# erincatto/solver2d

Hardware: AMD Instinct MI355X
Metric: contact-constraints x iters/sec, LargePyramid base-200 TGS_Soft (higher is better)
Workload: dtype f32

## Files before the change

include/solver2d_amd.h:

```cpp
#ifndef SOLVER2D_AMD_H
#define SOLVER2D_AMD_H

#include <stdint.h>

#ifdef __cplusplus
extern "C" {
#endif

#define S2AMD_API_VERSION 5

#define S2AMD_OK 0
#define S2AMD_E_INVALID (-1)
#define S2AMD_E_DEVICE (-2)
#define S2AMD_E_NODEVICE (-3)
#define S2AMD_E_STATE (-4)
#define S2AMD_E_CAPACITY (-5)

typedef enum s2amdSolverType
{
	s2amd_solverJacobi = 0,
	s2amd_solverPGS = 1,
	s2amd_solverPGS_NGS = 2,
	s2amd_solverPGS_NGS_Block = 3,
	s2amd_solverPGS_Soft = 4,
// ... 178 lines not shown
	uint16_t id[2];
	uint8_t cacheIndexA[3];
	uint8_t cacheIndexB[3];
	uint8_t persisted[2];
	uint8_t pad[2];
} s2amdPairState;

#define S2AMD_PAIR_UPDATED 0
#define S2AMD_PAIR_SEPARATED 1
#define S2AMD_PAIR_FREE (-1)

int s2amd_update_contacts(s2amdSolver* solver, const s2amdBody* bodies, int32_t bodyCapacity, const float* origins, const s2amdShape* shapes,
						  int32_t shapeCapacity, s2amdPairState* pairs, s2amdContact* contacts, int32_t contactCapacity, int32_t* status);

typedef struct s2amdWorldStepInfo
{
	int32_t separatedCount;
	int32_t activeContacts;
	int32_t graphChanged;
	int32_t movedCount;
	float contactsMs;
	float solveMs;
	float stepMs;
} s2amdWorldStepInfo;

int s2amd_world_upload(s2amdSolver* solver, const s2amdBody* bodies, int32_t bodyCapacity, const s2amdContact* contacts, int32_t contactCapacity,
					   const s2amdJoint* joints, int32_t jointCapacity, const s2amdShape* shapes, int32_t shapeCapacity, const s2amdPairState* pairs,
					   const float* origins);
int s2amd_world_step(s2amdSolver* solver, const s2amdStepParams* params, s2amdWorldStepInfo* info);
int s2amd_world_find_pairs(s2amdSolver* solver, int32_t* outPairs, int32_t pairCapacity, int32_t* pairCount);
int s2amd_world_separated(s2amdSolver* solver, int32_t* slots, int32_t capacity, int32_t* count);
typedef struct s2amdShapeBox
{
	float aabb[4];
	float fatAABB[4];
	int32_t enlarged;
} s2amdShapeBox;
int s2amd_world_download_boxes(s2amdSolver* solver, s2amdShapeBox* boxes, int32_t shapeCapacity);
typedef struct s2amdMovedBox
{
	int32_t shape;
	float fatAABB[4];
} s2amdMovedBox;
int s2amd_world_set_refit_order(s2amdSolver* solver, const int32_t* shapeOrder, int32_t count);
int s2amd_world_download_step(s2amdSolver* solver, float* poses, int32_t bodyCapacity, s2amdMovedBox* moved, int32_t movedCapacity, int32_t* movedCount);
typedef struct s2amdTreeNode
{
	float aabb[4];
	uint32_t categoryBits;
	int32_t parent;
	int32_t child1, child2;
	int32_t userData;
	int16_t height;
	uint8_t enlarged;
	uint8_t pad[9];
} s2amdTreeNode;
int s2amd_world_set_tree(s2amdSolver* solver, int32_t bodyType, const s2amdTreeNode* nodes, int32_t nodeCapacity, int32_t root);
int s2amd_world_get_tree(s2amdSolver* solver, int32_t bodyType, s2amdTreeNode* nodes, int32_t nodeCapacity, int32_t* root);
int s2amd_world_set_contacts(s2amdSolver* solver, const int32_t* slots, int32_t count, const s2amdContact* contacts, const s2amdPairState* pairs);
int s2amd_world_download(s2amdSolver* solver, s2amdBody* bodies, int32_t bodyCapacity, s2amdContact* contacts, int32_t contactCapacity,
						 s2amdJoint* joints, int32_t jointCapacity, s2amdShape* shapes, int32_t shapeCapacity, s2amdPairState* pairs, float* origins,
						 int32_t* status);

int s2amd_find_islands(s2amdSolver* solver, const s2amdBody* bodies, int32_t bodyCapacity, const s2amdContact* contacts, int32_t contactCapacity,
					   const s2amdJoint* joints, int32_t jointCapacity, int32_t* islandOfBody, int32_t* islandCount);
int s2amd_color_constraints(s2amdSolver* solver, const s2amdBody* bodies, int32_t bodyCapacity, const s2amdContact* contacts, int32_t contactCapacity,
							int32_t* colorOfContact, int32_t* colorCount, int32_t* rounds);

int s2amd_export_poses(s2amdSolver* solver, void* devicePoses, int32_t capacity);
int s2amd_export_poses_async(s2amdSolver* solver, void* devicePoses, int32_t capacity, int32_t slot);
int s2amd_export_bodies_async(s2amdSolver* solver, void* deviceRecords, int32_t capacity, int32_t slot);
int s2amd_export_wait(s2amdSolver* solver, int32_t slot);

int s2amd_device_alloc(s2amdSolver* solver, uint64_t bytes, void** devicePtr);
int s2amd_device_free(s2amdSolver* solver, void* devicePtr);
int s2amd_device_read(s2amdSolver* solver, void* hostDst, const void* deviceSrc, uint64_t bytes);

int s2amd_get_contact_order(s2amdSolver* solver, int32_t* order, int32_t orderCapacity, int32_t* colorOffsets,
							int32_t colorCapacity, int32_t* constraintCount, int32_t* colorCount);
int s2amd_get_joint_order(s2amdSolver* solver, int32_t* order, int32_t orderCapacity, int32_t* colorOffsets,
						  int32_t colorCapacity, int32_t* jointCount, int32_t* colorCount);
int s2amd_get_writable_bodies(s2amdSolver* solver, uint8_t* writable, int32_t bodyCapacity, int32_t* solverClass);
int s2amd_get_stats(s2amdSolver* solver, s2amdStepStats* stats);
int s2amd_get_strip_owners(s2amdSolver* solver, int32_t* ownerStrip, int32_t* onSeam, int32_t capacity, int32_t* stripCount);
int s2amd_measure_dominant(s2amdSolver* solver, const s2amdStepParams* params, int32_t repeats, float* usPerLaunch,
						   int32_t* launchesPerSweep, int32_t* constraintsPerLaunch);
int s2amd_set_option(s2amdSolver* solver, const char* key, int32_t value);

typedef struct s2amdShardedSolver s2amdShardedSolver;
int s2amd_sharded_create(const int32_t* devices, int32_t deviceCount, s2amdShardedSolver** out);
void s2amd_sharded_destroy(s2amdShardedSolver* sharded);
int s2amd_sharded_shard_count(const s2amdShardedSolver* sharded);
s2amdSolver* s2amd_sharded_solver(s2amdShardedSolver* sharded, int32_t shard);
int s2amd_sharded_upload(s2amdShardedSolver* sharded, const s2amdBody* bodies, int32_t bodyCapacity, const s2amdContact* contacts, int32_t contactCapacity,
						 const s2amdJoint* joints, int32_t jointCapacity);
int s2amd_sharded_step(s2amdShardedSolver* sharded, const s2amdStepParams* params);
int s2amd_sharded_step_async(s2amdShardedSolver* sharded, const s2amdStepParams* params);
int s2amd_sharded_wait(s2amdShardedSolver* sharded);
int s2amd_sharded_get_step_ops(s2amdShardedSolver* sharded, int32_t* streamOps, int32_t* hostWaits, int32_t* exchange);
int s2amd_sharded_count_ops(int32_t shards, int32_t exchange, int32_t* streamOps);
int s2amd_sharded_download(s2amdShardedSolver* sharded, s2amdBody* bodies, int32_t bodyCapacity, s2amdContact* contacts, int32_t contactCapacity,
						   s2amdJoint* joints, int32_t jointCapacity);
int s2amd_sharded_read_bodies(s2amdShardedSolver* sharded, int32_t shard, float* records, int32_t bodyCapacity);
int s2amd_sharded_reshard(s2amdShardedSolver* sharded, const s2amdContact* contacts, int32_t contactCapacity, const s2amdJoint* joints, int32_t jointCapacity);
int s2amd_sharded_get_partition(s2amdShardedSolver* sharded, int32_t* shardOfBody, int32_t capacity, int32_t* islandCount, int32_t* reshards);

#ifdef __cplusplus
}
#endif

#endif
```

solver2d_amd/csrc/launch.h:

```cpp
#pragma once

#include <hip/hip_runtime.h>

#include "solver2d_amd.h"

struct BodyView;
struct ContactView;
struct JointView;
struct JointPrepArgs;
struct Stage4Args;
struct StepConsts;
struct GroupTable;
struct Op;
struct MsgView;
struct StripTableView;
struct StripOps;
struct PersistView;
struct JacobiView;
struct s2amdBody;
struct s2amdContact;
struct s2amdJoint;
struct s2amdShape;
struct s2amdPairState;

// ... 56 lines not shown
						   int contactCapacity, const int* gatherIndex, const JointPrepArgs* joints = nullptr);
void launchWarmStartContacts(hipStream_t s, int kind, const ContactView& c, const BodyView& b, int begin, int end);
void launchSolveContactsSoft(hipStream_t s, int kind, const ContactView& c, const BodyView& b, int begin, int end, float inv_h, int useBias);
void launchSolveContactsRigid(hipStream_t s, int kind, const ContactView& c, const BodyView& b, int begin, int end, float inv_h);
void launchSolveContactsSticky(hipStream_t s, const ContactView& c, const BodyView& b, s2amdContact* wire, int begin, int end, float inv_h,
							   int useBias);
void launchSolveContactsNGS(hipStream_t s, const ContactView& c, const BodyView& b, int begin, int end);
void launchXpbdContactPositions(hipStream_t s, const ContactView& c, const BodyView& b, int begin, int end, float h);
void launchXpbdContactVelocities(hipStream_t s, const ContactView& c, const BodyView& b, int begin, int end, float h);
void launchBlockSolveVelocity(hipStream_t s, const ContactView& c, const BodyView& b, int begin, int end);
void launchBlockSolvePosition(hipStream_t s, const ContactView& c, const BodyView& b, int begin, int end);
bool launchStoreImpulses(hipStream_t s, int kind, const ContactView& c, s2amdContact* wire, float scale, const BodyView& bodies, s2amdBody* wireBodies,
						 void* clear, size_t clearBytes, const unsigned int* stepFailed, int finalizeMode = -1, const JointView* joints = nullptr,
						 s2amdJoint* wireJoints = nullptr,
						 const Stage4Args* stage4 = nullptr);

bool launchUnpackBodies(hipStream_t s, const BodyView& b, const s2amdBody* wire, const uint32_t* hostFlags, const StepConsts& sc, float h,
						s2amdContact* wireContacts, int contactCapacity, const int* gatherIndex, const JointPrepArgs* joints = nullptr, int posSolver = 0);
void launchPackBodies(hipStream_t s, const BodyView& b, s2amdBody* wire);
void launchIntegrateVelocities(hipStream_t s, const BodyView& b);
void launchIntegratePositions(hipStream_t s, const BodyView& b, float h);
void launchFinalizePositions(hipStream_t s, const BodyView& b, int dynamicOnly);
void launchJacobiApply(hipStream_t s, const BodyView& b, const ContactView& c, const int2* adjRange, const int* adjList, const int* heavy, int heavyCapacity);
void launchPatchWords(hipStream_t s, const void* devicePatches, int n);
void launchOverflowSweep(hipStream_t s, const Op& o, const ContactView& c, const BodyView& b, int begin, int end);
void launchXpbdIntegrate(hipStream_t s, const BodyView& b, float h);
void launchXpbdProject(hipStream_t s, const BodyView& b, float inv_h);
void launchExportPoses(hipStream_t s, const s2amdBody* wire, int n, void* out, int withVelocities = 0);

void launchPrepareJoints(hipStream_t s, int kind, const JointView& j, const uint32_t* hostFlags, const s2amdJoint* wire, const s2amdBody* wireBodies,
						 const StepConsts& sc, float h, float hertz, int warmStart, int posSolver);
void launchSolveJoints(hipStream_t s, int kind, const JointView& j, const BodyView& b, int begin, int end, const StepConsts& sc, float h,
					   float inv_h, int useBias);
void launchStoreJoints(hipStream_t s, const JointView& j, s2amdJoint* wire, const unsigned int* stepFailed);

int groupKernelSetup();
void launchGroupKernel(hipStream_t s, const ContactView& c, const JointView& j, const BodyView& g, const GroupTable& gt, const Op* ops, int opCount,
					   const StepConsts& sc, s2amdContact* wire, int maxBodies, int useDq0);
void launchStripKernel(hipStream_t s, const ContactView& c, const JointView& j, const BodyView& g, const GroupTable& gt, const Op* ops, int opCount,
					   const StepConsts& sc, s2amdContact* wire, int maxBodies, int useDq0);

void launchFillMessageSlots(hipStream_t s, const ContactView& c, const BodyView& b, const MsgView& m, int count);
void launchWarmStartContactsMsg(hipStream_t s, int kind, const ContactView& c, const MsgView& m, int begin, int end);
void launchSolveContactsSoftMsg(hipStream_t s, int kind, const ContactView& c, const MsgView& m, int begin, int end, float inv_h, int useBias);
void launchSolveContactsRigidMsg(hipStream_t s, int kind, const ContactView& c, const MsgView& m, int begin, int end, float inv_h);
void launchSolveContactsStickyMsg(hipStream_t s, const ContactView& c, const MsgView& m, s2amdContact* wire, int begin, int end, float inv_h,
								  int useBias);
void launchIntegrateVelocitiesMsg(hipStream_t s, const BodyView& b, const MsgView& m);
void launchIntegratePositionsMsg(hipStream_t s, const BodyView& b, const MsgView& m, float h);
void launchFinalizePositionsMsg(hipStream_t s, const BodyView& b, const MsgView& m, int dynamicOnly);
void launchGatherMessageSlots(hipStream_t s, const BodyView& b, const MsgView& m);

void launchWarmStartJointsBodies(hipStream_t s, const JointView& j, const BodyView& b, const int2* adjRange, const int* adjList);
void launchWarmStartBodies(hipStream_t s, int kind, const ContactView& c, const BodyView& b, const int2* adjRange, const int* adjList,
						   int integrateFirst, const int* heavy, int heavyCount);

int stripKernelSetup();
void launchIslandStep(hipStream_t s, int kind, int warm, const ContactView& c, const BodyView& g, const StripTableView& t, const float4* softCoef, const Op* ops,
					  int opCount, int maxRounds, s2amdContact* wire, const s2amdBody* wireBodies, const uint32_t* hostFlags, int warmStart,
					  const unsigned int* stepFailed);
void launchStripSoft(hipStream_t s, int kind, int warm, const ContactView& c, const BodyView& g, const StripTableView& t, const StripOps& ops);
void launchStripStep(hipStream_t s, int kind, int warm, const ContactView& c, const BodyView& g, const StripTableView& a, const PersistView& pv,
					 const Op* ops, int opCount);

int pairKernelSetup();
void launchPairStep(hipStream_t s, int kind, int warm, const ContactView& c, const BodyView& g, const StripTableView& a, const PersistView& pv, const Op* ops,
					int opCount);

int wideKernelSetup();
struct WideSelf
{
	s2amdContact* wire;
	s2amdBody* wireBodies;
	const uint32_t* hostFlags;
	int warmStart;
	float gravityX, gravityY, unpackH;
};
int wideExtraRecords(const PersistView& pv, int selfContained, int bodyWarm, int kind = SOFT_TGS);
int wideBodyWarmVariant(const PersistView& pv);
int wideIslandLocalRecords(int maxRounds);
void launchWideIsland(hipStream_t s, const ContactView& c, const BodyView& g, const StripTableView& t, const float4* softCoef, const Op* ops, int opCount,
					  int maxRounds, s2amdContact* wire, s2amdBody* wireBodies, const uint32_t* hostFlags, int warmStart, const StepConsts& sc, float unpackH,
					  int selfContained, const unsigned int* stepFailed, int allTwoPoints);
void launchWideStep(hipStream_t s, int kind, const ContactView& c, const BodyView& g, const StripTableView& a, const PersistView& pv, const Op* ops, int opCount,
					const WideSelf* self);

int jacobiKernelSetup();
size_t jacobiStepLds(int owned, int imports, int constraints, int opCount);
void launchJacobiStep(hipStream_t s, const ContactView& c, const JointView& jv, const BodyView& g, const JacobiView& t, const Op* ops, int opCount, const StepConsts& sc,
					  size_t ldsBytes, int maxConstraints);

int genericKernelSetup();
size_t genericStepLds(int bodies, int seamBodies, int exports, int opCount, int useDq0, int stagedJoints = 0);
void launchGenericStep(hipStream_t s, const ContactView& c, const JointView& j, const BodyView& g, const GroupTable& a, const GroupTable& b, const PersistView& pv,
					   const Op* ops, int opCount, const StepConsts& sc, s2amdContact* wire, int useDq0, int seamContacts, int seamJoints, size_t ldsBytes,
					   int stageJoints);

void launchUpdateContacts(hipStream_t st, const s2amdBody* bodies, const float* origins, const s2amdShape* shapes, s2amdPairState* pairs,
						  s2amdContact* contacts, int contactCapacity, int32_t* status, uint8_t* pointBytes, int* summary, int* separatedSlots, const uint8_t* watched);
void launchStage4(hipStream_t st, s2amdBody* bodies, int bodyCapacity, s2amdShape* shapes, int shapeCapacity, float* origins, int* summary,
				  const unsigned int* stepFailed = nullptr);
struct TreeView
{
	s2amdTreeNode* nodes;
	int* flag;
	int* leaves;
	int* state;
	int capacity;
	int *acc, *pending, *oldPre, *leafIdx, *partner, *arrive;
	float *cx, *cy;
	int *tasks, *ready, *qstate;
};
struct TreeViews
{
	TreeView t[3];
	const int* refitPos;
};
struct DeviceTrees;
void treesFree(s2amdSolver* s);
void treesForget(s2amdSolver* s);
bool treesActive(const s2amdSolver* s);
const TreeViews* treesViews(const s2amdSolver* s);
int treesSyncRefitOrder(s2amdSolver* s);
int worldWarmPairQuery(s2amdSolver* s);
void launchTreeEnlarge(s2amdSolver* s, hipStream_t st, const unsigned int* stepFailed);
void launchTreeRebuild(s2amdSolver* s, hipStream_t st);
void treesJoin(s2amdSolver* s, hipStream_t st);
void launchOrderPairs(hipStream_t st, const TreeViews* views, const s2amdShape* shapes, const unsigned char* moved, const unsigned long long* keys,
					  const unsigned int* count, unsigned int cap, unsigned long long* ckeys, unsigned long long* out);
struct PairQueryGraph
{
	hipGraphExec_t exec = nullptr;
	unsigned long long key = 0, keySeen = 0;
	bool disabled = false;
	char* host = nullptr;
	void* countAt = nullptr;
	size_t outCapWanted = 0;
};
struct PairQueryHook
{
	void (*fn)(void* arg, hipStream_t st);
	void* arg;
};
int findPairsResident(hipStream_t st, const s2amdShape* shapes, int shapeCapacity, int liveShapes, const s2amdPairState* pairs, int contactCapacity,
					  const unsigned long long* jointed, int jointedCount, int32_t* outPairs, int32_t pairCapacity, int32_t* pairCount, void** scratch,
					  size_t* scratchBytes, unsigned long long* sortedPairKeys, bool* sortedPairKeysValid, PairQueryGraph* cache, int mode = 0,
					  const unsigned long long* pairLog = nullptr, const int* pairLogSlots = nullptr, const TreeViews* trees = nullptr,
					  const PairQueryHook* hook = nullptr);
#define S2_PAIR_LOG_ENTRIES 255
#define S2_PAIRS_FULL 0
#define S2_PAIRS_WARM 1
#define S2_PAIRS_ENQUEUE 2
#define S2_PAIRS_COLLECT 3

#define S2_DEFINE_WARM(name)                                                                                                     \
	__global__ void s2WarmKernel_##name() {}                                                                                    \
	void s2Warm_##name(hipStream_t st) { s2WarmKernel_##name<<<dim3(1), dim3(64), 0, st>>>(); }
void s2Warm_contact_kernels(hipStream_t st);
void s2Warm_body_kernels(hipStream_t st);
void s2Warm_joint_kernels(hipStream_t st);
void s2Warm_group_kernel(hipStream_t st);
void s2Warm_strip_kernel(hipStream_t st);
void s2Warm_pair_kernel(hipStream_t st);
void s2Warm_wide_kernel(hipStream_t st);
void s2Warm_generic_kernel(hipStream_t st);
void s2Warm_broadphase(hipStream_t st);
void s2Warm_narrowphase(hipStream_t st);
// ... 7 lines not shown
```

solver2d_amd/csrc/s2_device.h:

```cpp
#pragma once

#include <hip/hip_runtime.h>
#include <stdint.h>

#define S2_DEV __device__ __forceinline__

#define S2_PI 3.14159265359f
#define S2_LINEAR_SLOP 0.005f
#define S2_ANGULAR_SLOP (2.0f / 180.0f * S2_PI)
#define S2_MAX_LINEAR_CORRECTION 0.2f
#define S2_MAX_ANGULAR_CORRECTION (8.0f / 180.0f * S2_PI)
#define S2_BAUMGARTE 0.2f
#define S2_MAX_BAUMGARTE_VELOCITY 4.0f
#define S2_CONTACT_HERTZ 30.0f
#define S2_JOINT_HERTZ 60.0f

#define S2_MINF(A, B) ((A) < (B) ? (A) : (B))
#define S2_MAXF(A, B) ((A) > (B) ? (A) : (B))
#define S2_ABSF(A) ((A) > 0.0f ? (A) : -(A))
#define S2_CLAMPF(A, B, C) S2_MINF(S2_MAXF(A, B), C)

struct V2
{
	float x, y;
// ... 391 lines not shown
struct GroupTable
{
	const int* bodyOffsets;
	const int* bodyIds;
	const int* cBatchOffsets;
	const int4* cBatches;
	const int* jBatchOffsets;
	const int4* jBatches;
	int groupCount;
};
#define S2G_OWNED 0x80000000u

#define S2_STRIP_ROUNDS 6
#define S2_STRIP_ROUNDS_MAX 8
#define S2_STRIP_BODY_CHUNKS 4
struct StripDesc
{
	int bodyBase, bodyCount, ownedCount;
	int batchCount;
	int slotBase, slotCount, slotOffBase;
	int pad;
	int4 batch[S2_STRIP_ROUNDS_MAX];
};
struct StripOps
{
	int integratePos, integrateVel, sweep, useBias;
	float posH, inv_h;
};
struct StripTableView
{
	const StripDesc* descs;
	const int* bodyIds;
	const int2* slots;
	const int* slotOffsets;
	int groupCount;
	int ldsRecords;
};

#define S2_PERSIST_B_ROUNDS 4
#define S2_PERSIST_Q_NARROW 6
#define S2_PERSIST_Q_WIDE 8
struct PersistDesc
{
	int importCount[2];
	int importIdBase[2];
	int exportCount[2];
	int exportSrcBase[2];
	int inBase[2];
	int outBase[2];
	int remapBase[2];
	int seamBatchCount[2];
	int2 seamBatch[2][S2_PERSIST_B_ROUNDS];
	int seamGroup[2];
	int pad[6];
};
struct PersistView
{
	const PersistDesc* descs;
	const int* remap;
	const int* exportSrc;
	const int* importIds;
	unsigned long long* granules;
	unsigned int* error;
	unsigned int* deviceError;
	int parityStride;
	int censusBase;
	int allTwoPoints;
	float4 softCoef[2];
	int wideRounds;
	int seamRegs;
	int maxRoundsA, maxSeamRounds;
	int pairLanes;
	int nearHandoff;
	int wideOnly;
	int ldsRecords;
	int parkSeamWidth, parkInteriorWidth;
	int bodyRecords;
	int debugSkip;
	unsigned int spinLimit;
	unsigned int* state;
	int maxStaged;
	int maxStripBodies;
	int bodyWarm;
	int clearOwn;
	const int* overflowBodies;
	int overflowBodyCount;
	int overflowBegin, overflowEnd;
	int overflowGranBase;
	int overflowKernel;
	unsigned long long* debugTimes;
};
#define S2_OVERFLOW_BODIES 64
#define S2_OVERFLOW_RING 4
#define S2_OVERFLOW_GRANULES (2 * S2_OVERFLOW_RING * S2_OVERFLOW_BODIES * 4)

#define S2_JACOBI_HEAVY 32
struct JacobiBlockDesc
{
	int ownedBase, ownedCount;
	int importBase, importCount;
	int constraintBase, constraintCount;
	int listBase, rangeBase;
	int exportBase, exportCount;
	int heavyBase, heavyCount;
	int jointBase, jointCount;
};
struct JacobiView
{
	const JacobiBlockDesc* descs;
	const int* ints;
	unsigned long long* granules;
	int parityStride;
	unsigned int* error;
	unsigned int* deviceError;
	unsigned int spinLimit;
	int blockCount;
	int debugSkip;
};

struct MsgView
{
	float4* vel;
	float4* dq;
	const int* next;
	const int* firstSlot;
	const int* slotOffsets;
	const int* slotList;
};
```

solver2d_amd/csrc/solver.cpp:

```cpp

#include <atomic>
#include "solver_executor.h"

namespace
{

thread_local std::string g_lastError;

}

int s2amdFail(int code, const std::string& msg)
{
	g_lastError = msg;
	return code;
}

hipStream_t s2amdStream(s2amdSolver* s)
{
	return s->stream;
}
void s2amdRecordDeviceMs(s2amdSolver* s, float ms)
{
	s->stats.deviceMs = ms;
}
// ... 553 lines not shown
		return fail(S2AMD_E_CAPACITY, "the solver holds " + std::to_string(s->hBodyFlags.size()) + " bodies");
	}
	const int cls = s->orderSolverClass == 1 ? 1 : 0;
	const uint32_t bit = cls == 1 ? S2F_WRITE_POS : S2F_WRITE_VEL;
	for (size_t i = 0; i < s->hBodyFlags.size(); ++i)
	{
		writable[i] = (s->hBodyFlags[i] & bit) != 0 ? 1 : 0;
	}
	if (solverClass)
	{
		*solverClass = cls;
	}
	return S2AMD_OK;
}

int s2amd_get_joint_order(s2amdSolver* s, int32_t* order, int32_t orderCapacity, int32_t* colorOffsets, int32_t colorCapacity, int32_t* jointCount,
						  int32_t* colorCount)
{
	if (!s)
	{
		return fail(S2AMD_E_INVALID, "null solver");
	}
	return copyOrder(s->joints.order, s->joints.colorOffsets, order, orderCapacity, colorOffsets, colorCapacity, jointCount, colorCount);
}

int s2amd_get_strip_owners(s2amdSolver* s, int32_t* ownerStrip, int32_t* onSeam, int32_t capacity, int32_t* stripCount)
{
	if (!s)
	{
		return fail(S2AMD_E_INVALID, "null solver");
	}
	const IncrementalStrips& m = s->stripInc;
	const int nb = s->bodyCapacity;
	if ((ownerStrip || onSeam) && capacity < nb)
	{
		return fail(S2AMD_E_CAPACITY, "strip owner buffer too small");
	}
	if (stripCount)
	{
		*stripCount = m.valid ? (int)m.stripBodyCount.size() : 0;
	}
	for (int i = 0; i < nb; ++i)
	{
		if (ownerStrip)
		{
			ownerStrip[i] = (m.valid && i < (int)m.ownerStrip.size()) ? m.ownerStrip[(size_t)i] : -1;
		}
		if (onSeam)
		{
			onSeam[i] = -1;
		}
	}
	if (onSeam && m.valid)
	{
		for (size_t sm = 0; sm < m.seamGroupOf.size(); ++sm)
		{
			const int g = m.seamGroupOf[sm];
			if (g < 0)
			{
				continue;
			}
			for (const auto& kv : m.seamSlot[(size_t)g])
			{
				if (kv.first >= 0 && kv.first < nb && m.ownerStrip[(size_t)kv.first] >= 0)
				{
					onSeam[kv.first] = (int)sm;
				}
			}
		}
	}
	return S2AMD_OK;
}

int s2amd_get_stats(s2amdSolver* s, s2amdStepStats* stats)
{
	if (!s || !stats)
	{
		return fail(S2AMD_E_INVALID, "null argument");
	}
	*stats = s->stats;
	return S2AMD_OK;
}

int s2amd_export_poses(s2amdSolver* s, void* devicePoses, int32_t capacity)
{
	if (!s || !s->resident)
	{
		return fail(S2AMD_E_STATE, "nothing resident");
	}
	if (!devicePoses || capacity < s->bodyCapacity)
	{
		return fail(S2AMD_E_CAPACITY, "pose buffer missing or too small");
	}
	HIP_TRY(hipSetDevice(s->device));
	launchExportPoses(s->stream, (const s2amdBody*)s->dBodies.p, s->bodyCapacity, devicePoses);
	HIP_TRY(hipGetLastError());
	HIP_TRY(hipStreamSynchronize(s->stream));
	return S2AMD_OK;
}

int s2amd_export_poses_async(s2amdSolver* s, void* devicePoses, int32_t capacity, int32_t slot)
{
	if (!s || !s->resident)
	{
		return fail(S2AMD_E_STATE, "nothing resident");
	}
	if (!devicePoses || capacity < s->bodyCapacity || slot < 0 || slot >= 4)
	{
		return fail(S2AMD_E_CAPACITY, "pose buffer missing or too small, or slot outside 0..3");
	}
	HIP_TRY(hipSetDevice(s->device));
	if (!s->evExport[slot])
	{
		HIP_TRY(hipEventCreateWithFlags(&s->evExport[slot], hipEventDisableTiming));
	}
	launchExportPoses(s->stream, (const s2amdBody*)s->dBodies.p, s->bodyCapacity, devicePoses);
	HIP_TRY(hipGetLastError());
	HIP_TRY(hipEventRecord(s->evExport[slot], s->stream));
	return S2AMD_OK;
}

int s2amd_export_bodies_async(s2amdSolver* s, void* deviceRecords, int32_t capacity, int32_t slot)
{
	if (!s || !s->resident)
	{
		return fail(S2AMD_E_STATE, "nothing resident");
	}
	if (!deviceRecords || capacity < s->bodyCapacity || slot < 0 || slot >= 4)
	{
		return fail(S2AMD_E_CAPACITY, "record buffer missing or too small, or slot outside 0..3");
	}
	HIP_TRY(hipSetDevice(s->device));
	if (!s->evExport[slot])
	{
		HIP_TRY(hipEventCreateWithFlags(&s->evExport[slot], hipEventDisableTiming));
	}
	launchExportPoses(s->stream, (const s2amdBody*)s->dBodies.p, s->bodyCapacity, deviceRecords, 1);
	HIP_TRY(hipGetLastError());
	HIP_TRY(hipEventRecord(s->evExport[slot], s->stream));
	return S2AMD_OK;
}

int s2amd_export_wait(s2amdSolver* s, int32_t slot)
{
	if (!s || slot < 0 || slot >= 4 || !s->evExport[slot])
	{
		return fail(S2AMD_E_STATE, "no export recorded in this slot");
	}
	HIP_TRY(hipSetDevice(s->device));
	HIP_TRY(hipEventSynchronize(s->evExport[slot]));
	return S2AMD_OK;
}

int s2amd_device_alloc(s2amdSolver* s, uint64_t bytes, void** devicePtr)
{
	if (!s || !devicePtr)
	{
		return fail(S2AMD_E_INVALID, "null argument");
	}
	*devicePtr = nullptr;
	HIP_TRY(hipSetDevice(s->device));
	HIP_TRY(hipMalloc(devicePtr, bytes > 0 ? (size_t)bytes : 16));
	HIP_TRY(hipMemsetAsync(*devicePtr, 0, bytes > 0 ? (size_t)bytes : 16, s->stream));
	HIP_TRY(hipStreamSynchronize(s->stream));
	return S2AMD_OK;
}
// ... 266 lines not shown
	}
	else if (strcmp(key, "strip_retry") == 0)
	{
		s->optStripRetry = value != 0;
		s->structureDirty = true;
	}
	else if (strcmp(key, "persist") == 0)
	{
		s->stripsRejected = false;
		s->optPersist = value != 0;
		s->structureDirty = true;
	}
	else if (strcmp(key, "strip_patience") == 0)
	{
		s->optStripPatience = std::max(0, value);
		s->stripPatienceNow = s->optStripPatience;
		s->stripPatienceSet = true;
	}
	else if (strcmp(key, "near_handoff") == 0)
	{
		s->optNearHandoff = value != 0;
		s->nearHandoffNow = s->optNearHandoff;
	}
	else if (strcmp(key, "strip_adopt") == 0)
	{
		s->optStripAdopt = value != 0;
	}
	else if (strcmp(key, "prebuild_solver") == 0)
	{
		s->optPrebuildSolver = value;
	}
	else if (strcmp(key, "jacobi_persist") == 0)
	{
		s->optJacobiPersist = value != 0;
		s->structureDirty = true;
	}
	else if (strcmp(key, "jacobi_min_constraints") == 0)
	{
		s->optJacobiMinConstraints = std::max(0, value);
		s->structureDirty = true;
	}
	else if (strcmp(key, "strip_overflow") == 0)
	{
		s->optOverflow = value != 0;
		s->structureDirty = true;
	}
	else if (strcmp(key, "cost_strip_round_ns") == 0 || strcmp(key, "cost_launch_ns") == 0 || strcmp(key, "cost_tail_visit_ns") == 0)
	{
		float& f = key[5] == 's' ? s->hubCosts.stripRoundUs : (key[5] == 'l' ? s->hubCosts.launchUs : s->hubCosts.tailVisitUs);
		f = 1e-3f * (float)std::max(value, 1);
		s->structureDirty = true;
	}
	else if (strcmp(key, "tree_stream") == 0)
	{
		s->optTreeStream = value != 0 ? 1 : 0;
	}
	else if (strcmp(key, "pairs_in_step") == 0)
	{
		s->optPairsInStep = value != 0;
		s->pairCacheValid = false;
	}
	else if (strcmp(key, "overflow_kernel") == 0)
	{
		s->optOverflowKernel = value != 0;
		s->overflowKernelFailed = false;
		s->layoutGeneration += 1;
	}
	else if (strcmp(key, "stage_joints") == 0)
	{
		s->optStageJoints = value != 0;
	}
	else if (strcmp(key, "step_readback") == 0)
	{
		s->optStepReadback = value != 0;
	}
	else if (strcmp(key, "self_contained") == 0)
	{
		s->optSelfContained = value != 0;
	}
	else if (strcmp(key, "strip_body_warm") == 0)
	{
		s->optWideBodyWarm = value != 0;
	}
	else if (strcmp(key, "self_contained_strips") == 0)
	{
		if (s->optSelfContainedStrips != (value != 0 ? 1 : 0))
		{
			s->structureDirty = true;
		}
		s->optSelfContainedStrips = value != 0;
	}
	else if (strcmp(key, "free_body_groups") == 0)
	{
		s->optFreeBodyGroups = value != 0;
		s->structureDirty = true;
	}
	else if (strcmp(key, "persist_retry") == 0)
	{
		s->optPersistRetry = std::max(0, value);
		s->persistRetryAfter = std::max(1, value);
	}
	else if (strcmp(key, "generic") == 0)
	{
		s->stripsRejected = false;
		s->optGeneric = value != 0;
		s->structureDirty = true;
	}
	else if (strcmp(key, "strips_any_solver") == 0)
	{
		s->stripsRejected = false;
		s->optStripsAnySolver = value != 0;
		s->structureDirty = true;
	}
	else if (strcmp(key, "island_resident") == 0)
	{
		s->optIslandResident = value != 0;
		s->residentRejected = false;
		s->structureDirty = true;
	}
	else if (strcmp(key, "incremental") == 0)
	{
		s->optIncremental = value != 0;
		s->structureDirty = true;
	}
	else if (strcmp(key, "defer") == 0)
	{
		s->optDefer = value != 0;
		s->structureDirty = true;
	}
	else if (strcmp(key, "strip_lean") == 0)
	{
		s->stripsRejected = false;
		s->optStripLean = value != 0;
		s->structureDirty = true;
	}
	else if (strcmp(key, "strip_bodies") == 0)
	{
		s->stripsRejected = false;
		s->optStripBodies = std::max(1, value);
		s->stripBodiesSet = true;
		s->structureDirty = true;
	}
	else if (strcmp(key, "strip_min_bodies") == 0)
	{
		s->stripsRejected = false;
		s->optStripMinBodies = std::max(0, value);
		s->stripMinBodiesSet = true;
		s->structureDirty = true;
	}
	else if (strcmp(key, "pack_group_bodies") == 0)
	{
		s->optPackGroupBodies = std::max(1, value);
		s->packGroupBodiesSet = true;
		s->structureDirty = true;
	}
	else
	{
		return fail(S2AMD_E_INVALID, std::string("unknown option ") + key);
	}
	return S2AMD_OK;
}

}
#pragma GCC visibility pop
```

solver2d_amd/csrc/solver_executor.h:

```cpp
#pragma once

#include "solver_internal.h"


struct Executor
{
	s2amdSolver* s;
	hipStream_t st;
	const StepPlan& p;
	int posSolver;
	bool profile;
	bool msg = false;
	bool fork = false;
	const int* gatherIndex = nullptr;

	hipStream_t branch(int i, int forkEvent)
	{
		if (!fork)
		{
			return st;
		}
		(void)hipEventRecord(s->evFork[forkEvent], st);
		(void)hipStreamWaitEvent(s->side[i], s->evFork[forkEvent], 0);
		return s->side[i];
// ... 336 lines not shown
				continue;
			}
			if (o.code == OP_WARM && (o.kind == WARM_CURRENT || o.kind == WARM_FIXED) && (warm < 0 || warm == o.kind))
			{
				warm = o.kind;
				continue;
			}
			if (leanSoftKind(o) && (kind < 0 || kind == o.kind))
			{
				kind = o.kind;
				continue;
			}
			return false;
		}
		if (kind < 0)
		{
			return false;
		}
		if (warm < 0)
		{
			warm = kind == SOFT_FIXED ? WARM_FIXED : WARM_CURRENT;
		}
		if (widePlan(kind, warm))
		{
			return true;
		}
		if (s->persist.wideOnly)
		{
			return false;
		}
		const bool narrow = kind == SOFT_TGS && warm == WARM_CURRENT;
		const int records = (narrow ? s->persist.ldsRecords : s->persistRecordsWide) + 2 * (int)p.ops.size();
		return records <= (160 * 1024) / 16;
	}

	bool genericPlan() const
	{
		if (!s->genericValid || s->persistFailed || p.ops.size() > 128)
		{
			return false;
		}
		for (const Op& o : p.ops)
		{
			if (o.code == OP_JACOBI_APPLY || (o.code == OP_SOLVE_SOFT && o.kind == SOFT_JACOBI))
			{
				return false;
			}
		}
		return genericStepLds(s->genericBodies, s->genericSeamBodies, s->genericExports, (int)p.ops.size(), p.usesDq0 ? 1 : 0) <= 160 * 1024;
	}

	bool oneLaunchPlan() const
	{
		int kind, warm;
		return persistPlan(kind, warm) || genericPlan();
	}

	bool widePlan(int kind, int warm) const
	{
		const bool current = (kind == SOFT_TGS || kind == SOFT_PGS) && warm == WARM_CURRENT;
		const bool fixed = kind == SOFT_FIXED && warm == WARM_FIXED;
		return s->optWide && (current || fixed) && wideFits(false, false, kind);
	}

	bool wideFits(bool selfContained, bool bodyWarm, int kind = SOFT_TGS) const
	{
		const int extra = wideExtraRecords(s->persist, selfContained ? 1 : 0, bodyWarm ? 1 : 0, kind);
		return extra >= 0 && s->persist.bodyRecords + 3 + extra + 2 * s->persistOpCount <= (160 * 1024) / 16;
	}

	bool selfContainedStrips() const
	{
		int kind, warm;
		return s->optSelfContainedStrips && !slicedPlan() && s->dStripA.view.groupCount > 0 && persistPlan(kind, warm) && kind == SOFT_TGS && widePlan(kind, warm) && wideFits(true, false) && gatherIndex == nullptr && !msg &&
			   wireBodies() != nullptr && s->dGroups.view.groupCount == 0 && s->dResident.view.groupCount == 0 && s->looseBodies == 0 && !anyGlobalContacts() &&
			   s->joints.globalCount == 0 && s->jv.count == 0 && s->cv.count == s->persistK1 - s->persistK0 && p.prepContacts == PREP_SOFT && p.storeKind == STORE_PLAIN;
	}

	bool wideBodyWarm(bool selfContained) const
	{
		return s->optWideBodyWarm != 0 && wideBodyWarmVariant(s->persist) != 0 && wideFits(selfContained, true);
	}

	bool residentPlan(int& kind, int& warm) const
	{
		kind = -1, warm = -1;
		if (s->residentView.groupCount <= 0 || p.ops.size() > 128 || p.prepContacts != PREP_SOFT || p.storeKind != STORE_PLAIN)
		{
			return false;
		}
		if (s->dStripA.view.groupCount > 0 && oneLaunchPlan())
		{
			return false;
		}
		for (const Op& o : p.ops)
		{
			if (o.code == OP_INTEGRATE_VEL || o.code == OP_INTEGRATE_POS || o.code == OP_FINALIZE || o.code == OP_JOINT_SWEEP)
			{
				continue;
			}
			if (o.code == OP_WARM && (o.kind == WARM_CURRENT || o.kind == WARM_FIXED) && (warm < 0 || warm == o.kind))
			{
				warm = o.kind;
				continue;
			}
			if (leanSoftKind(o) && (kind < 0 || kind == o.kind))
			{
				kind = o.kind;
				continue;
			}
			return false;
		}
		if (kind < 0)
		{
			return false;
		}
		if (warm < 0)
		{
			warm = kind == SOFT_FIXED ? WARM_FIXED : WARM_CURRENT;
		}
		return true;
	}

	int uploadResidentOps()
	{
		if (s->residentOpsGeneration == s->planGeneration)
		{
			return 0;
		}
		std::vector<Op> kept;
		for (const Op& o : p.ops)
		{
			if (o.code != OP_JOINT_SWEEP)
			{
				kept.push_back(o);
			}
		}
		bool grew = false;
		int rc = s->dResidentOps.ensure(std::max<size_t>(kept.size(), 1) * sizeof(Op), &grew);
		if (rc)
		{
			return rc;
		}
		if (grew)
		{
			s->layoutGeneration += 1;
		}
		if (hipMemcpyAsync(s->dResidentOps.p, kept.data(), kept.size() * sizeof(Op), hipMemcpyHostToDevice, st) != hipSuccess ||
			hipStreamSynchronize(st) != hipSuccess)
		{
			return S2AMD_E_DEVICE;
		}
		s->residentOpCount = (int)kept.size();
		s->residentOpsGeneration = s->planGeneration;
		return 0;
	}

	bool wideIslandPlan() const
	{
		int kind, warm;
		return residentPlan(kind, warm) && s->optWide && kind == SOFT_TGS && warm == WARM_CURRENT &&
			   s->residentView.ldsRecords + 2 + wideIslandLocalRecords(s->residentRounds) + 2 * s->residentOpCount <= (160 * 1024) / 16;
	}

	bool selfContainedIslands() const
	{
// ... 21 lines not shown
			{
				launchWideIsland(st, s->cv, s->bv, s->residentView, coef, (const Op*)s->dResidentOps.p, s->residentOpCount, s->residentRounds, wireContacts(),
								 wireBodies(), (const uint32_t*)s->dBodyFlags.p, p.sc.warmStart, p.sc, p.unpackH, selfContained ? 1 : 0, stepFailed,
								 (s->residentAllTwoPoints && s->pointsKnown) ? 1 : 0);
			}
			else
			{
				launchIslandStep(st, kind, warm, s->cv, s->bv, s->residentView, coef, (const Op*)s->dResidentOps.p, s->residentOpCount, s->residentRounds,
								 wireContacts(), wireBodies(), (const uint32_t*)s->dBodyFlags.p, p.sc.warmStart, stepFailed);
			}
		}
		else
		{
			launchGroupKernel(st, s->cv, s->jv, s->bv, s->dResident.view, deviceOps(), (int)p.ops.size(), p.sc, wireContacts(), s->dResident.maxBodies,
							  p.usesDq0 ? 1 : 0);
		}
		count();
	}

	int uploadPersistOps()
	{
		if (s->persistOpsGeneration == s->planGeneration && s->persistOpsStructure == s->structureGeneration)
		{
			return 0;
		}
		std::vector<Op> kept;
		for (const Op& o : p.ops)
		{
			if (!sweepsNothing(o))
			{
				kept.push_back(o);
			}
		}
		bool grew = false;
		int rc = s->dPersistOps.ensure(std::max<size_t>(kept.size(), 1) * sizeof(Op), &grew);
		if (rc)
		{
			return rc;
		}
		if (grew)
		{
			s->layoutGeneration += 1;
		}
		if (hipMemcpyAsync(s->dPersistOps.p, kept.data(), kept.size() * sizeof(Op), hipMemcpyHostToDevice, st) != hipSuccess ||
			hipStreamSynchronize(st) != hipSuccess)
		{
			return S2AMD_E_DEVICE;
		}
		s->persistOpCount = (int)kept.size();
		s->persistOpsGeneration = s->planGeneration;
		s->persistOpsStructure = s->structureGeneration;
		return 0;
	}

	std::vector<Op> keptOps() const
	{
		std::vector<Op> kept;
		for (const Op& o : p.ops)
		{
			if (!sweepsNothing(o))
			{
				kept.push_back(o);
			}
		}
		return kept;
	}

	bool slicedPlan() const { return s->stripInc.valid && s->stripInc.overflowUsed > 0; }

	void runPersistentSliced(int kind, int warm)
	{
		const std::vector<Op> kept = keptOps();
		const int n = (int)kept.size();
		PersistView pv = s->persist;
		pv.nearHandoff = s->nearHandoffNow;
		for (int i = 0; i < 2; ++i)
		{
			pv.softCoef[i] = make_float4(p.sc.softCoef[i][0], p.sc.softCoef[i][1], p.sc.softCoef[i][2], 0.0f);
		}
		if (!(kind == SOFT_TGS && warm == WARM_CURRENT))
		{
			pv.ldsRecords = s->persistRecordsWide;
		}
		pv.bodyWarm = 0;
		pv.clearOwn = 1;
		const IncrementalStrips& m = s->stripInc;
		int first = 0;
		for (int i = 0; i < n; ++i)
		{
			const Op& o = kept[(size_t)i];
			const bool sweep = o.code == OP_WARM || leanSoftKind(o);
			if (!sweep && i + 1 < n)
			{
				continue;
			}
			launchWideStep(st, kind, s->cv, s->bv, s->leanA, pv, (const Op*)s->dPersistOps.p + first, i + 1 - first, nullptr);
			count();
			if (sweep)
			{
				launchOverflowSweep(st, o, s->cv, s->bv, m.overflowBegin, m.overflowEnd);
				count();
			}
			first = i + 1;
		}
	}

	void clearGranules(hipStream_t where)
	{
		(void)hipMemsetAsync(s->dGranules.p, 0, s->granuleBytes, where);
		count();
	}

	bool overflowKernelPlan() const
	{
		return slicedPlan() && s->optOverflowKernel != 0 && !s->overflowKernelFailed && s->persist.overflowBodies != nullptr && s->dStripA.view.groupCount + 1 <= s->cuCount;
	}

	void runPersistent(int kind, int warm, bool clearFirst = false, bool selfContained = false, bool overflowKernel = false)
	{
		if (clearFirst)
		{
			clearGranules(st);
		}
		if (profile)
		{
			recordEvent();
		}
		PersistView pv = s->persist;
		pv.nearHandoff = s->nearHandoffNow;
		for (int i = 0; i < 2; ++i)
		{
			pv.softCoef[i] = make_float4(p.sc.softCoef[i][0], p.sc.softCoef[i][1], p.sc.softCoef[i][2], 0.0f);
		}
		if (!(kind == SOFT_TGS && warm == WARM_CURRENT))
		{
			pv.ldsRecords = s->persistRecordsWide;
		}
		if (widePlan(kind, warm))
		{
			WideSelf self{};
			if (selfContained)
			{
				self.wire = wireContacts(), self.wireBodies = wireBodies(), self.hostFlags = (const uint32_t*)s->dBodyFlags.p;
				self.warmStart = p.sc.warmStart, self.gravityX = p.sc.gravityX, self.gravityY = p.sc.gravityY, self.unpackH = p.unpackH;
			}
			pv.bodyWarm = (kind == SOFT_TGS && wideBodyWarm(selfContained)) ? 1 : 0;
			if (overflowKernel)
			{
				const IncrementalStrips& m = s->stripInc;
				pv.bodyWarm = 0;
				pv.overflowKernel = 1;
				pv.overflowBodyCount = (int)m.overflowBodyIds.size();
				pv.overflowBegin = m.overflowBegin, pv.overflowEnd = m.overflowEnd;
			}
			launchWideStep(st, kind, s->cv, s->bv, s->leanA, pv, (const Op*)s->dPersistOps.p, s->persistOpCount, selfContained ? &self : nullptr);
		}
		else if (pv.pairLanes && s->optPairLanes)
		{
			launchPairStep(st, kind, warm, s->cv, s->bv, s->leanA, pv, (const Op*)s->dPersistOps.p, s->persistOpCount);
		}
		else
		{
			launchStripStep(st, kind, warm, s->cv, s->bv, s->leanA, pv, (const Op*)s->dPersistOps.p, s->persistOpCount);
		}
		if (profile)
		{
			recordEvent();
		}
		count();
	}

	void runGeneric()
	{
		if (profile)
		{
			recordEvent();
		}
		const size_t withJoints = genericStepLds(s->genericBodies, s->genericSeamBodies, s->genericExports, s->persistOpCount, p.usesDq0 ? 1 : 0, s->genericJoints);
		const bool stage = s->optStageJoints != 0 && s->genericJoints > 0 && withJoints <= 160 * 1024;
		const size_t lds = stage ? withJoints : genericStepLds(s->genericBodies, s->genericSeamBodies, s->genericExports, s->persistOpCount, p.usesDq0 ? 1 : 0);
		PersistView gpv = s->persist;
		gpv.nearHandoff = s->nearHandoffNow;
		launchGenericStep(st, s->cv, s->jv, s->bv, s->dStripA.view, s->dStripB.view, gpv, (const Op*)s->dPersistOps.p, s->persistOpCount, p.sc,
						  wireContacts(), p.usesDq0 ? 1 : 0, s->contacts.seamCount > 0 ? 1 : 0, s->joints.seamCount > 0 ? 1 : 0, lds, stage ? 1 : 0);
		if (profile)
		{
			recordEvent();
		}
		count();
	}

	void runStrips()
	{
		int kind, warm;
		if (persistPlan(kind, warm))
		{
			if (slicedPlan() && widePlan(kind, warm))
			{
				if (overflowKernelPlan())
				{
					runPersistent(kind, warm, false, false, true);
				}
				else
				{
					runPersistentSliced(kind, warm);
				}
			}
			else
			{
				runPersistent(kind, warm);
			}
			return;
		}
		if (genericPlan())
		{
			runGeneric();
			return;
		}
		const int n = (int)p.ops.size();
		int segStart = 0;
		for (int i = 0; i < n; ++i)
		{
			const Op& o = p.ops[(size_t)i];
			if (isBodyOp(o.code) || sweepsNothing(o))
			{
				continue;
			}
			StripOps lean;
			int warm = -1;
			if (o.code == OP_WARM)
			{
				int j = i + 1;
				while (j < n && (isBodyOp(p.ops[(size_t)j].code) || sweepsNothing(p.ops[(size_t)j])))
				{
					j += 1;
				}
				if (j < n && leanSegment(segStart, j, lean, warm) && warm >= 0)
				{
// ... 224 lines not shown
```

solver2d_amd/csrc/solver_internal.h:

```cpp
#pragma once

#include "launch.h"
#include "s2_device.h"

#include "solver2d_amd.h"

#include <algorithm>
#include <chrono>
#include <cmath>
#include <cstdio>
#include <cstdlib>
#include <cstring>
#include <string>
#include <unordered_map>
#include <vector>

int s2amdFail(int code, const std::string& msg);
inline int fail(int code, const std::string& msg) { return s2amdFail(code, msg); }

#define S2_HUB_DEGREE 12
#define S2_COST_STRIP_ROUND_US 1.4f
#define S2_COST_LAUNCH_US 2.0f
#define S2_COST_BATCH_COLOURS 12
#define S2_COST_TAIL_VISIT_US 0.38f
// ... 200 lines not shown
	bool takeOnly = false;
	std::vector<int> stripBodyBase, stripBodyCount;
	std::vector<int> stripListCapacity;
	std::vector<std::vector<int>> movedList;
	std::vector<int> adoptedBy;
	int spareIdsNext = 0, spareIdsEnd = 0;
	long adopted = 0;
	std::vector<int> seamBodyCount;
	std::vector<int> seamExtra[2];
	long seamBodiesAdded = 0;
	int overflowBegin = 0, overflowEnd = 0;
	std::vector<int> overflowFree;
	int overflowUsed = 0;
	long overflowPlaced = 0;
	std::vector<int> overflowBodyIds;
};
#define S2_OVERFLOW_SLACK 32
#define S2_STRIP_ADOPT_SLACK 8
#define S2_TAIL_SLACK 64
#define S2_GROUP_PATIENCE_MIN_POSITIONS 16384
#define S2_TAIL_BODY_SLACK 32

struct SolverStructure
{
	std::vector<int> hContactA, hContactB;
	std::vector<uint8_t> hContactEdge;
	std::vector<uint8_t> hContactDead;
	std::vector<uint8_t> hBodyHub, hContactWatched;
	int watchedCount = 0;
	DevBuf dWatched;
	std::vector<uint32_t> hBodyFlagsFinal;
	std::vector<uint8_t> hBodyLdsOwned;
	DevBuf dBodyFlags;

	DevBuf soaBodies, soaContacts, soaJoints, dContactIndex, dJointIndex, dContactLocal, dJointLocal, dAdjOffsets, dAdjList, dAdjHeavy;
	int adjHeavyCapacity = 0;
	IncrementalGlobal inc;
	uint4* hostPatches = nullptr;
	size_t hostPatchCapacity = 0;
	DevBuf dPatches;
	int spareColours = 0;
	DevBuf dJointAdjRange, dJointAdjList;
	bool jointAdjValid = false;
	int slackPositions = 0;
	bool slackBumped = false;
	int slackAtBuild = 0;
	int slackShift = 0;
	const char* dirtyReason = "";
	bool watchedDirty = false;
	BodyView bv{};
	ContactView cv{};
	JointView jv{};
	uint64_t layoutGeneration = 0;
	int bodySoaCap = 0, contactSoaCap = 0, jointSoaCap = 0;

	SweepSet contacts, joints;
	HostGroupTable hGroups, hContactTail, hJointTail, hStripA, hStripB;
	std::vector<int> hPersistRemap;
	std::vector<PersistDesc> hPersistDescs;
	DeviceGroupTable dGroups, dContactTail, dJointTail, dStripA, dStripB;
	HostGroupTable hResident;
	DeviceGroupTable dResident;
	DevBuf dResidentDesc, dResidentOps;
	StripTableView residentView{};
	int residentRounds = 0;
	int residentK0 = 0, residentK1 = 0;
	bool residentRejected = false;
	uint64_t residentOpsGeneration = ~0ull;
	int residentOpCount = 0;
	DevBuf dStripLean;
	StripTableView leanA{}, leanB{};
	bool leanAValid = false, leanBValid = false;
	DevBuf dPersist, dGranules, dOverflowBodies;
	PersistView persist{};
	bool persistValid = false;
	bool genericValid = false;
	int genericJoints = 0;
	int genericBodies = 0, genericSeamBodies = 0, genericExports = 0;
	int residentAllTwoPoints = 0;
	int persistK0 = 0, persistK1 = 0;
	int persistRecordsWide = 0;
	DevBuf dPersistOps;
	int persistOpCount = 0;
	DevBuf dJacobi, dJacobiGran;
	JacobiView jacobi{};
	int jacobiDeferred = 0;
	bool jacobiValid = false;
	size_t jacobiGranBytes = 0;
	int jacobiMaxOwned = 0, jacobiMaxImports = 0, jacobiMaxConstraints = 0;
	uint64_t persistOpsGeneration = ~0ull, persistOpsStructure = ~0ull;
	size_t granuleBytes = 0;
	long selfStepsSinceReset = 0;
	IncrementalStrips stripInc;
	float stripScaleFound = 0.0f;
	bool stripRetryPending = false;
	DevBuf dMsg;
	MsgView msg{};
	bool msgTablesValid = false;
	int looseBodies = 0;
	int orderSolverClass = -1;
	bool orderGrouped = false;
	bool orderLdsGroups = false;
	bool orderResident = false;
	bool orderColourless = false;
	bool orderStrips = false;
	int orderStripBodies = 0;
	bool stripsNeedOneLaunch = false;
	bool stripsRejected = false;
	int stripsJudgedForClass = -1;
	bool stripsHopeless = false;
	bool adjValid = false;
	bool structureDirty = true;
	uint64_t structureGeneration = 0;
	int stripScaleFoundFor = 0;

	hipGraph_t graph = nullptr;
	hipGraphExec_t graphExec = nullptr;
	uint64_t graphKey = 0;
	uint64_t graphKeySeen = 0;
	int graphKeySeenLaunches = 0;
	int graphLaunches = 0;
};

struct AsyncBuild;

struct SolverRest
{
	int device = 0;
	hipStream_t stream = nullptr;
	hipEvent_t evBegin = nullptr, evEnd = nullptr;
	hipEvent_t evExport[4] = {nullptr, nullptr, nullptr, nullptr};
	hipStream_t side[2] = {nullptr, nullptr};
	hipEvent_t evFork[2] = {nullptr, nullptr}, evJoin[4] = {nullptr, nullptr, nullptr, nullptr};
	int optAsync = 0;
	bool constraintIndexInPrologue = false;
	int optFork = 0;

	DevBuf dBodies, dContacts, dJoints, dBodiesSaved;
	int bodyCapacity = 0, contactCapacity = 0, jointCapacity = 0;
	bool resident = false;
	bool savedValid = false;
	int savedBodyCapacity = 0;

	DevBuf dShapes, dPairs, dOrigins, dStatus, dPointBytes, dWorldSummary, dJointedKeys, dContactStage, dPairScratch, dPairKeys;
	PairQueryGraph pairQuery;
	bool pairKeysValid = false;
	int shapeCapacity = 0, liveShapes = 0, jointedCount = 0;
	bool worldResident = false;
	int* hostWorldSummary = nullptr;
	uint8_t* hostSlotStage = nullptr;
	size_t hostSlotStageBytes = 0;
	char* hostStepBack = nullptr;
	size_t hostStepBackBytes = 0, stepBackPoseOffset = 0;
	int stepBackBoxes = 0;
	bool stepBackValid = false;
	bool stepBackListFresh = false;
	int optStepReadback = 1;
	std::vector<uint8_t> hPointBytes;
	std::vector<uint8_t> hShapeMovable;
	int movableShapes = 0;
	std::vector<int> hContactPoints;
	bool deadUnknown = false;
	bool pointsKnown = false;
	bool pointCountsFresh = false;
	int optPrebuildSolver = -1;
	int activeContacts = 0;
	bool lastStepWroteIndex = false;
	DevBuf dScanTmp;
	std::vector<int> hJointType, hJointA, hJointB;
	std::vector<uint32_t> hBodyFlags;
	std::vector<uint8_t> hBodyLive, hBodyStatic;
	DevBuf dOps;
	long placedTotal = 0;
	DevBuf dSeparated;
	DevBuf dPairLog;
	unsigned long long* hostPairLog = nullptr;
	bool pairLogDirty = false;
	DevBuf dShapeBoxes;
	DevBuf dRefitOrder, dStepBack;
	int refitOrderCount = 0;
	int optTreeStream = 1;
	DeviceTrees* trees = nullptr;
	int lastMovedCount = 0;
	DevBuf dSlotBytes;
	std::vector<uint8_t> hSlotBytes;
	bool slotBytesFresh = false;
	std::vector<int32_t> hSeparated;
	int optIncremental = 1;
	int optDefer = 1;
	int optIslandResident = 1;
	int optStripLean = 1;
	int optStageJoints = 1;
	int optSelfContained = 1;
	int optGeneric = 1;
	int optFreeBodyGroups = 1;
	int optPersist = 1;
	int optSeamRegs = 1;
	int optWide = 1;
	int optWideBodyWarm = 0;
	int optSelfContainedStrips = 0;
	int optStripSlack = 1;
	int optPairLanes = 0;
	int optStripRetry = 1;
	int optPersistDebug = 0;
	int optPersistSpinLimit = 1 << 21;
	bool persistFailed = false;
	int persistFallbacks = 0;
	int optPersistRetry = 256;
	int persistRetryAfter = 256, persistFailedAge = 0;
	int cuCount = 0;
	HubCosts hubCosts;
	unsigned int* hostError = nullptr;
	unsigned long long* hostTimes = nullptr;
	int optMessage = 0;
	int optBodyWarm = 1;
	bool indexInWire = false;
	int graphAge = 0;
	int optStripPatience = 1;
	int optNearHandoff = 1, nearHandoffNow = 1, nearHandoffTimeouts = 0;
	int optStripAdopt = 1;
	int optJacobiPersist = 1;
	int optJacobiMinConstraints = 1024;
	int optOverflow = 1;
	long slicedSteps = 0;
	bool slicedThisStep = false;
	int stripPatienceNow = 1;
	int groupPatienceNow = 0;
	bool dirtyByGroups = false;
	int tailSlackShift = 0;
	bool dirtyByWatched = false;
	int optGroupPatience = 1;
	int optTailTinyColour = 32;
	int optGroupTinyColour = 3;
	int optGenericPlace = 1;
	int optFlipColours = 1;
	bool stripPatienceSet = false;
	int optStripsAnySolver = 0;

	StepPlan plan;
	uint64_t planGeneration = 0;

	int optGraph = 1;
	int optGraphMinLaunches = 6;
	int optProfile = 0;
	int optGroups = 1;
	int optMaxGroupBodies = 1024;
	bool maxGroupBodiesSet = false;
	int optPackGroupBodies = 1024;
	bool packGroupBodiesSet = false;
	int optStrips = 1;
	int optStripBodies = 8;
	bool stripBodiesSet = false;
	int optStripBodiesLds = 320;
	bool stripMinBodiesSet = false;
	int optStripMinBodies = 768;

	std::vector<hipEvent_t> sweepEvents;
	size_t sweepEventsUsed = 0;

	s2amdStepStats stats{};
	int launchCounter = 0;
	DevBuf dGatherIndex;
	bool gatherIndexDirty = true;
	uint64_t opsGeneration = ~0ull;

	AsyncBuild* async = nullptr;
	int optAsyncBuild = 1;
	int optAsyncBuildDelay = 12;
	bool isClone = false;
	bool poolWarmed = false;
	bool forcedBuild = false;
	Stage4Args stage4{};
	bool stage4Carried = false;
	bool graphCarriesStage4 = false;
	int optPairsInStep = 1;
	bool pairQueryUsed = false;
	bool pairCacheValid = false;
	int optOverflowKernel = 1;
	bool overflowKernelFailed = false;
	bool overflowKernelThisStep = false;
	int overflowRefusals = 0;
	long stepCounter = 0;
// ... 120 lines not shown
```

solver2d_amd/csrc/solver_step.cpp:

```cpp
#include "solver_executor.h"

void destroyGraph(s2amdSolver* s)
{
	if (s->graphExec)
	{
		(void)hipGraphExecDestroy(s->graphExec);
		s->graphExec = nullptr;
	}
	if (s->graph)
	{
		(void)hipGraphDestroy(s->graph);
		s->graph = nullptr;
	}
	s->graphKey = 0;
}

int resetPersistState(s2amdSolver* s, hipStream_t st)
{
	if (s->hostError)
	{
		*s->hostError = 0u;
	}
	if (s->persist.deviceError)
	{
// ... 575 lines not shown
		}
		if ((key != s->graphKey || s->graphExec == nullptr) && (key != s->graphKeySeen || s->graphKeySeenLaunches < s->optGraphMinLaunches))
		{
			s->graphKeySeen = key;
			q.fork = false;
			enqueueAll();
			s->graphKeySeenLaunches = s->launchCounter;
		}
		else if (key != s->graphKey || s->graphExec == nullptr)
		{
			destroyGraph(s);
			HIP_TRY(hipStreamBeginCapture(s->stream, hipStreamCaptureModeThreadLocal));
			enqueueAll();
			hipError_t ce = hipStreamEndCapture(s->stream, &s->graph);
			if (ce != hipSuccess)
			{
				s->graph = nullptr;
				return fail(S2AMD_E_DEVICE, std::string("hipStreamEndCapture: ") + hipGetErrorString(ce));
			}
			HIP_TRY(hipGraphInstantiate(&s->graphExec, s->graph, nullptr, nullptr, 0));
			s->graphKey = key;
			s->graphLaunches = s->launchCounter;
			s->graphCarriesStage4 = s->stage4Carried;
		}
		else
		{
			s->launchCounter = s->graphLaunches;
			s->stats.graphReplayed = 1;
			s->stage4Carried = s->graphCarriesStage4;
		}
		if (key == s->graphKey && s->graphExec != nullptr)
		{
			HIP_TRY(hipGraphLaunch(s->graphExec, s->stream));
		}
	}
	else
	{
		enqueueAll();
	}
	HIP_TRY(hipEventRecord(s->evEnd, s->stream));
	HIP_TRY(hipGetLastError());
	s->indexInWire = s->indexInWire || indexNow;
	const bool async = s->optAsync != 0 && !q.profile;
	if (!async)
	{
		HIP_TRY(hipStreamSynchronize(s->stream));
		float ms = 0.0f;
		HIP_TRY(hipEventElapsedTime(&ms, s->evBegin, s->evEnd));
		s->stats.deviceMs = ms;
	}
	s->stats.constraintCount = s->activeContacts;
	s->stats.jointCount = s->jv.count;
	s->stats.contactColors = (int)s->contacts.colorOffsets.size() - 1;
	s->stats.jointColors = (int)s->joints.colorOffsets.size() - 1;
	s->stats.solveSweeps = plan.solveSweeps;
	s->stats.kernelLaunches = s->launchCounter;
	s->stats.groupCount = s->dGroups.view.groupCount + s->dResident.view.groupCount;
	s->stats.stripCount = s->dStripA.view.groupCount;
	s->stats.seamCount = s->dStripB.view.groupCount;
	{
		int kind, warm;
		s->stats.persistent = ((s->dStripA.view.groupCount > 0 && (q.persistPlan(kind, warm) || q.genericPlan())) || q.jacobiPlan()) ? 1 : 0;
	}
	s->stats.persistFallbacks = s->persistFallbacks;
	s->stats.asyncBuildsRequested = s->asyncRequested, s->stats.asyncBuildsAdopted = s->asyncAdopted, s->stats.asyncWaitMs = s->asyncWaitMs;
	s->stats.nearHandoffTimeouts = s->nearHandoffTimeouts;
	{
		int kind, warm;
		s->slicedThisStep = s->dStripA.view.groupCount > 0 && q.slicedPlan() && q.persistPlan(kind, warm) && q.widePlan(kind, warm) && !q.selfContainedStrips();
		s->overflowKernelThisStep = s->slicedThisStep && q.overflowKernelPlan();
		s->slicedSteps += s->slicedThisStep ? 1 : 0;
		s->stats.overflowContacts = s->stripInc.valid ? s->stripInc.overflowUsed : 0;
		s->stats.slicedStep = s->slicedThisStep ? (s->overflowKernelThisStep ? 2 : 1) : 0;
		s->stats.slicedSteps = (int32_t)s->slicedSteps;
	}
	s->stats.bodiesAdopted = (int32_t)s->stripInc.adopted, s->stats.seamBodiesAdded = (int32_t)s->stripInc.seamBodiesAdded, s->stats.roundsOpened = (int32_t)s->stripInc.roundsOpened;
	s->stats.structureBuilds = (int32_t)s->structureGeneration;
	s->stats.placedContacts = (int32_t)s->placedTotal;
	{
		int kind = -1, warm = -1;
		const bool persistent = s->stats.persistent && q.persistPlan(kind, warm);
		const bool wide = persistent && q.widePlan(kind, warm);
		s->stats.pairLanes = wide ? 2 : (persistent && s->persist.pairLanes && s->optPairLanes) ? 1 : (s->stats.persistent && !persistent) ? 3 : 0;
	}
	s->stats.potentialConstraints = (int32_t)(s->contacts.order.size() - (size_t)s->slackPositions);
	if (!async && s->hostError && *s->hostError != 0u)
	{
		int rcReset = resetPersistState(s, s->stream);
		if (rcReset)
		{
			return rcReset;
		}
		if (s->nearHandoffNow != 0 && s->stats.persistent)
		{
			s->nearHandoffNow = 0;
			s->nearHandoffTimeouts += 1;
			s->layoutGeneration += 1;
			s->stepCounter -= 1;
			return doStep(s, params);
		}
		if (s->overflowKernelThisStep && !s->overflowKernelFailed)
		{
			s->overflowKernelFailed = true;
			s->layoutGeneration += 1;
			s->persistFallbacks += 1;
			s->stepCounter -= 1;
			return doStep(s, params);
		}
		s->persistFailed = true;
		s->persistFailedAge = 0;
		s->persistFallbacks += 1;
		s->stepCounter -= 1;
		return doStep(s, params);
	}
	s->graphAge += 1;
	if (q.profile)
	{
		float total = 0.0f;
		for (size_t i = 0; i + 1 < s->sweepEventsUsed; i += 2)
		{
			float t = 0.0f;
			if (hipEventElapsedTime(&t, s->sweepEvents[i], s->sweepEvents[i + 1]) == hipSuccess)
			{
				total += t;
			}
		}
		float empty = 0.0f;
		int pairs = 0;
		if (s->sweepEvents.size() >= 2)
		{
			for (int r = 0; r < 32; ++r)
			{
				(void)hipEventRecord(s->sweepEvents[0], s->stream);
				(void)hipEventRecord(s->sweepEvents[1], s->stream);
				(void)hipStreamSynchronize(s->stream);
				float t = 0.0f;
				if (hipEventElapsedTime(&t, s->sweepEvents[0], s->sweepEvents[1]) == hipSuccess)
				{
					empty += t;
					pairs += 1;
				}
			}
		}
		s->stats.solveKernelMs = total;
		s->stats.solveLaunches = (int)(s->sweepEventsUsed / 2);
		s->stats.eventPairOverheadMs = pairs > 0 ? empty / pairs : 0.0f;
	}
	return S2AMD_OK;
}

int doDownload(s2amdSolver* s, s2amdBody* bodies, int nb, s2amdContact* contacts, int nc, s2amdJoint* joints, int nj)
{
	if (!s->resident)
	{
		return fail(S2AMD_E_STATE, "nothing resident to download");
	}
	if (nb < s->bodyCapacity || nc < s->contactCapacity || nj < s->jointCapacity)
	{
		return fail(S2AMD_E_CAPACITY, "output arrays smaller than the resident world");
	}
	HIP_TRY(hipSetDevice(s->device));
	if (contacts && !s->pointsKnown && s->lastStepWroteIndex)
	{
		int rc = refreshConstraintIndexOnDevice(s);
		if (rc)
		{
// ... 20 lines not shown
```

solver2d_amd/csrc/wide_kernel.hip:

```cpp

#include "body_ops.h"
#include "persist_handoff.h"
#include "soft_from_wire.h"

#ifndef S2_PERSIST_INSTRUMENTED
#define S2_PERSIST_INSTRUMENTED 0
#endif
#ifndef S2_WIDE_XCD_AFFINE
#define S2_WIDE_XCD_AFFINE 1
#endif
#define S2_WIDE_THREADS 512
#define S2_WIDE_INTERIOR 256
#define S2_WIDE_ROUNDS_PER_HALF (S2_STRIP_ROUNDS / 2)
#define S2_WIDE_BODY_CHUNKS 2
#define S2_WIDE_SEAM_ROUNDS 2

typedef float f2 __attribute__((ext_vector_type(2)));

S2_DEV f2 lo2(float4 v) { return f2{v.x, v.y}; }
S2_DEV f2 hi2(float4 v) { return f2{v.z, v.w}; }
struct WideRegs
{
	uint32_t idx;
	f2 n;
// ... 375 lines not shown
			const float tangentMass = fromBits(asBits(p.p2[j]) ^ salt);
			const V2 rA = pre.rA[j], rB = pre.rB[j];
			const V2 vrB = add(vB, crossSV(wB, rB));
			const V2 vrA = add(vA, crossSV(wA, rA));
			const float vt = dot(sub(vrB, vrA), tangent);
			float impulse = -tangentMass * vt;
			const float maxFriction = p.friction * nImp[j];
			const float newImpulse = S2_CLAMPF(tImp[j] + impulse, -maxFriction, maxFriction);
			impulse = newImpulse - tImp[j];
			const V2 P = mulSV(impulse, tangent);
			vA = mulSub(vA, mA, P);
			wA -= iA * cross(rA, P);
			vB = mulAdd(vB, mB, P);
			wB += iB * cross(rB, P);
			p.imp[j] = f2{nImp[j], newImpulse};
		}
	}

	if ((idx & (1u << 28)) != 0)
	{
		lvel[ia] = make_float4(vA.x, vA.y, wA, 0.0f);
	}
	if ((idx & (1u << 29)) != 0)
	{
		lvel[ib] = make_float4(vB.x, vB.y, wB, 0.0f);
	}
}
#endif

S2_DEV void storeWide(const ContactView& c, const WideRegs& p, int k)
{
	const int pointCount = (int)((p.idx >> 26) & 3u);
#pragma unroll
	for (int j = 0; j < 2; ++j)
	{
		if (j < pointCount)
		{
			c.impulse[j][k] = make_float2(p.imp[j].x, p.imp[j].y);
		}
	}
}

#define S2_WIDE_PARKED_RECORDS 6
#ifndef S2_WIDE_PARKED_PREP_EARLY
#define S2_WIDE_PARKED_PREP_EARLY 0
#endif
S2_DEV void parkWide(float4* slot, int stride, const WideRegs& p)
{
	slot[0 * stride] = make_float4(fromBits(p.idx), p.n.x, p.n.y, p.friction);
	slot[1 * stride] = make_float4(p.lA[0].x, p.lA[0].y, p.lA[1].x, p.lA[1].y);
	slot[2 * stride] = make_float4(p.lB[0].x, p.lB[0].y, p.lB[1].x, p.lB[1].y);
	slot[3 * stride] = make_float4(p.p0[0], p.p0[1], p.p1[0], p.p1[1]);
	slot[4 * stride] = make_float4(p.p2[0], p.p2[1], 0.0f, 0.0f);
	slot[5 * stride] = make_float4(p.imp[0].x, p.imp[0].y, p.imp[1].x, p.imp[1].y);
}
S2_DEV WideRegs unparkWide(const float4* slot, int stride)
{
	const float4 q0 = slot[0 * stride], q1 = slot[1 * stride], q2 = slot[2 * stride], q3 = slot[3 * stride], q4 = slot[4 * stride], q5 = slot[5 * stride];
	WideRegs p;
	p.idx = asBits(q0.x), p.n = f2{q0.y, q0.z}, p.friction = q0.w;
	p.lA[0] = lo2(q1), p.lA[1] = hi2(q1), p.lB[0] = lo2(q2), p.lB[1] = hi2(q2);
	p.p0[0] = q3.x, p.p0[1] = q3.y, p.p1[0] = q3.z, p.p1[1] = q3.w, p.p2[0] = q4.x, p.p2[1] = q4.y;
	p.imp[0] = lo2(q5), p.imp[1] = hi2(q5);
	return p;
}

S2_DEV WideRegs wideFromSoft(const SoftRegs<SOFT_TGS>& t)
{
	WideRegs p;
	p.idx = (uint32_t)t.h.ia | ((uint32_t)t.h.ib << 13) | (((uint32_t)t.h.pointCount & 3u) << 26) | (t.h.writeA ? 1u << 28 : 0u) | (t.h.writeB ? 1u << 29 : 0u);
	p.n = f2{t.h.normal.x, t.h.normal.y}, p.friction = t.h.friction;
#pragma unroll
	for (int j = 0; j < 2; ++j)
	{
		p.lA[j] = lo2(t.an[j]), p.lB[j] = hi2(t.an[j]);
		p.p0[j] = t.par[j].x, p.p1[j] = t.par[j].y, p.p2[j] = t.par[j].z;
		p.imp[j] = f2{t.imp[j].x, t.imp[j].y};
	}
	return p;
}

#define S2_WIDE_SELF 1
#define S2_WIDE_BODYWARM 2
#define S2_WIDE_SLICED 4

template <int POINTS, bool LL = false>
S2_DEV void warmTermsWide(const WideRegs& p, const float4* ldq, const float2* lmass, float2* lt, int tw, int R, int round, int nOwn, uint32_t salt, const float4* locals = nullptr)
{
	const uint32_t idx = p.idx ^ salt;
	const int ia = (int)(idx & 0x1fffu), ib = (int)((idx >> 13) & 0x1fffu);
	const int pointCount = (int)((idx >> 26) & 3u);
	const bool wa = (idx & (1u << 28)) != 0 && ia < nOwn, wb = (idx & (1u << 29)) != 0 && ib < nOwn;
	const float4 dqA = ldq[ia], dqB = ldq[ib];
	const float2 mA = lmass[ia], mB = lmass[ib];
	const V2 normal = v2(fromBits(asBits(p.n.x) ^ salt), p.n.y);
	const V2 tangent = rightPerp(normal);
	Rot qA, qB;
	qA.s = dqA.z, qA.c = dqA.w, qB.s = dqB.z, qB.c = dqB.w;
	float tA[6], tB[6];
#pragma unroll
	for (int j = 0; j < 2; ++j)
	{
		tA[3 * j] = tA[3 * j + 1] = tA[3 * j + 2] = 0.0f;
		tB[3 * j] = tB[3 * j + 1] = tB[3 * j + 2] = 0.0f;
		if (POINTS == 2 || j < pointCount)
		{
			V2 lAj, lBj;
			if constexpr (LL)
			{
				const float4 a = locals[j * S2_WIDE_THREADS];
				lAj = v2(a.x, a.y), lBj = v2(a.z, a.w);
			}
			else
			{
				lAj = asV2(p.lA[j]), lBj = asV2(p.lB[j]);
			}
			const V2 rA = rotate(qA, lAj), rB = rotate(qB, lBj);
			const V2 P = add(mulSV(p.imp[j].x, normal), mulSV(p.imp[j].y, tangent));
			tA[3 * j] = -mA.x * P.x, tA[3 * j + 1] = -mA.x * P.y, tA[3 * j + 2] = -(mA.y * cross(rA, P));
			tB[3 * j] = mB.x * P.x, tB[3 * j + 1] = mB.x * P.y, tB[3 * j + 2] = mB.y * cross(rB, P);
		}
	}
	float2* row = lt + (size_t)round * tw;
	const int plane = R * tw;
	if (wa)
	{
		row[ia] = make_float2(tA[0], tA[1]);
		row[plane + ia] = make_float2(tA[2], tA[3]);
		row[2 * plane + ia] = make_float2(tA[4], tA[5]);
	}
	if (wb)
	{
		row[ib] = make_float2(tB[0], tB[1]);
		row[plane + ib] = make_float2(tB[2], tB[3]);
		row[2 * plane + ib] = make_float2(tB[4], tB[5]);
	}
}

constexpr int wideLocalsInLds(int RPH, int SR, int SL, int IL, bool sliced)
{
	const int plain = (SL > 0 || IL > 0) ? (IL > 0 ? 4 : 3) : ((RPH + SR > 5) ? 3 : 0);
	return plain > 0 && sliced ? plain + 1 : plain;
}

S2_DEV int wideOverflowExchange(const PersistView& pv, const int* lovf, float4* lvel, int ovCount, unsigned sweep)
{
	const int tid = (int)threadIdx.x;
	int fail = 0;
	if (tid < ovCount)
	{
		const int e = lovf[tid];
		if (e != 0)
		{
			const int slot = e & 0xffffff;
			gu64* in = (gu64*)pv.granules + pv.overflowGranBase + (int)(sweep & (S2_OVERFLOW_RING - 1)) * S2_OVERFLOW_BODIES * 4 + 4 * tid;
			gu64* out = in + S2_OVERFLOW_GRANULES / 2;
			if ((e >> 24) == 3)
			{
				const float4 v = lvel[slot];
				putGranule(in + 0, sweep, v.x), putGranule(in + 1, sweep, v.y), putGranule(in + 2, sweep, v.z);
			}
			float v[3];
			if (getGranules<3>(out, sweep, v, pv.error, pv.deviceError, pv.spinLimit))
			{
				lvel[slot] = make_float4(v[0], v[1], v[2], 0.0f);
			}
			else
			{
				fail = 1;
			}
		}
	}
	return __syncthreads_or(fail);
}

#define S2_WIDE_OVERFLOW 8

template <int KIND> S2_DEV void wideOverflowWorker(const ContactView& c, const BodyView& g, const PersistView& pv, const Op* ops, int opCount, float4* lds)
{
	const int tid = (int)threadIdx.x;
	const int M = pv.overflowBodyCount;
	__shared__ float4 lvel[S2_OVERFLOW_BODIES], ldq[S2_OVERFLOW_BODIES];
	Op* lops = (Op*)lds;
	uint32_t flags = 0u;
	bool exchanged = false;
	float4 vel = make_float4(0.0f, 0.0f, 0.0f, 0.0f), dq = vel, integ = vel;
	float angDamp = 0.0f;
	if (tid < M)
	{
		const int e = pv.overflowBodies[tid];
		if (e >= 0)
		{
			const int gi = e & 0x3fffffff;
			exchanged = (e & 0x40000000) == 0;
			vel = g.vel[gi], dq = g.dq[gi], integ = g.integ[gi], angDamp = g.angDamp[gi];
			flags = g.flags[gi];
		}
	}
	for (int i = tid; i < opCount * 8; i += S2_WIDE_THREADS)
	{
		((int*)lops)[i] = ((const int*)ops)[i];
	}
	const int myK = pv.overflowBegin + tid;
	const bool mine = tid < 64 && myK < pv.overflowEnd && c.contactIndex[myK] >= 0;
	__syncthreads();
	const LdsBodies lb{lvel, ldq};
	gu64* in = (gu64*)pv.granules + pv.overflowGranBase + 4 * tid;
	gu64* out = in + S2_OVERFLOW_GRANULES / 2;
	unsigned sweep = 0u;
	for (int oi = 0; oi < opCount; ++oi)
	{
		const Op op = lops[oi];
		if (op.code == OP_INTEGRATE_VEL)
		{
			if ((flags & S2F_DYNAMIC) != 0)
			{
				V2 lv = add(v2(vel.x, vel.y), v2(integ.x, integ.y));
				float w = vel.z + integ.z;
				lv = mulSV(integ.w, lv);
				w *= angDamp;
				vel = make_float4(lv.x, lv.y, w, 0.0f);
// ... 59 lines not shown
					__builtin_amdgcn_fence(__ATOMIC_RELEASE, "wavefront");
					__builtin_amdgcn_wave_barrier();
					__builtin_amdgcn_fence(__ATOMIC_ACQUIRE, "wavefront");
				}
			}
			__syncthreads();
			if (exchanged)
			{
				vel = lvel[tid];
				putGranule(out + ring + 0, sweep, vel.x), putGranule(out + ring + 1, sweep, vel.y), putGranule(out + ring + 2, sweep, vel.z);
			}
		}
		else if (op.code == OP_WARM)
		{
			WarmRegs w;
			if (mine)
			{
				w = op.kind == WARM_FIXED ? loadWarm<WARM_FIXED>(c, lb, myK) : loadWarm<WARM_CURRENT>(c, lb, myK);
			}
			sweep += 1u;
			const int ring = (int)(sweep & (S2_OVERFLOW_RING - 1)) * S2_OVERFLOW_BODIES * 4;
			int fail = 0;
			if (exchanged)
			{
				float v[3];
				if (getGranules<3>(in + ring, sweep, v, pv.error, pv.deviceError, pv.spinLimit))
				{
					vel = make_float4(v[0], v[1], v[2], 0.0f);
				}
				else
				{
					fail = 1;
				}
			}
			if (tid < M)
			{
				lvel[tid] = vel, ldq[tid] = dq;
			}
			if (__syncthreads_or(fail))
			{
				return;
			}
			if (tid < 64)
			{
				for (unsigned long long turns = __ballot(mine); turns != 0ull; turns &= turns - 1ull)
				{
					if (tid == __builtin_ctzll(turns))
					{
						if (op.kind == WARM_FIXED)
						{
							applyWarm<WARM_FIXED>(w, lb);
						}
						else
						{
							applyWarm<WARM_CURRENT>(w, lb);
						}
					}
					__builtin_amdgcn_fence(__ATOMIC_RELEASE, "wavefront");
					__builtin_amdgcn_wave_barrier();
					__builtin_amdgcn_fence(__ATOMIC_ACQUIRE, "wavefront");
				}
			}
			__syncthreads();
			if (exchanged)
			{
				vel = lvel[tid];
				putGranule(out + ring + 0, sweep, vel.x), putGranule(out + ring + 1, sweep, vel.y), putGranule(out + ring + 2, sweep, vel.z);
			}
		}
	}
}

template <int POINTS, int RPH, int SR, int SL = 0, int IL = 0, int MODE = 0, int KIND = SOFT_TGS> __global__ __launch_bounds__(S2_WIDE_THREADS) void wideStepKernel(ContactView c, BodyView g, StripTableView ta, PersistView pv, const Op* ops, int opCount, WideSelf self)
{
	extern __shared__ __attribute__((aligned(16))) float4 lds[];
	constexpr bool SELF = (MODE & S2_WIDE_SELF) != 0;
	constexpr bool BODYWARM = (MODE & S2_WIDE_BODYWARM) != 0;
	static_assert(!BODYWARM || (SL == 0 && IL == 0), "the body-centric warm start keeps no terms for parked rounds");
	constexpr bool SLICED = (MODE & S2_WIDE_SLICED) != 0;
	constexpr bool OVERFLOW = (MODE & S2_WIDE_OVERFLOW) != 0;
	static_assert(KIND == SOFT_TGS || (MODE & ~(S2_WIDE_SLICED | S2_WIDE_OVERFLOW)) == 0, "the self-contained form and the body-centric warm start are s2Solve_TGS_Soft's");
	static_assert(!SLICED || MODE == S2_WIDE_SLICED, "a sliced step's launches are the plain form");
	static_assert(!OVERFLOW || MODE == S2_WIDE_OVERFLOW, "the overflow workgroup rides with the plain form");
	if constexpr (OVERFLOW)
	{
		if (blockIdx.x + 1u == gridDim.x)
		{
			wideOverflowWorker<KIND>(c, g, pv, ops, opCount, lds);
			return;
		}
	}
	static_assert(KIND != SOFT_FIXED || (SL == 0 && IL == 0), "s2Solve_SoftStep: the variants without parked rounds");
	constexpr int RK = KIND == SOFT_PGS ? S2_WIDE_PGS_ARMS : KIND;
	constexpr int RKP = KIND;
	constexpr int NRES = RPH + SR;
	constexpr int LA = KIND == SOFT_TGS ? wideLocalsInLds(RPH, SR, SL, IL, SLICED || OVERFLOW) : 0;
	constexpr int LL0 = NRES - LA;
	static_assert(LA >= 0 && LA <= NRES, "wideLocalsInLds");
	const int tid = (int)threadIdx.x;
#ifndef S2_WIDE_SPREAD_HALVES
#define S2_WIDE_SPREAD_HALVES 0
#endif
#if S2_WIDE_SPREAD_HALVES
	const int half = (tid >> 7) & 1, ht = (tid & 127) | ((tid >> 8) << 7);
#else
	const int half = tid >> 8, ht = tid & 255;
#endif
	const bool stamp = S2_PERSIST_INSTRUMENTED && pv.debugTimes != nullptr && tid == 0 &&
					   blockIdx.x == (((pv.debugSkip >> 8) & 0xff) != 0 ? (unsigned)(((pv.debugSkip >> 8) & 0xff) - 1) : 8 * (gridDim.x / 16) + 3);
	int stamps = 0;
	auto stampAt = [&](unsigned tag) {
		if (stamp && stamps < 250)
		{
			pv.debugTimes[stamps++] = (wall_clock64() << 4) | tag;
		}
	};
	stampAt(0);
	const int K = (int)gridDim.x - (OVERFLOW ? 1 : 0);
	const int xcd = (int)blockIdx.x & 7, lane8 = (int)blockIdx.x >> 3;
	const int strip = S2_WIDE_XCD_AFFINE ? xcd * (K >> 3) + (xcd < (K & 7) ? xcd : (K & 7)) + lane8 : (int)blockIdx.x;
	const int firstOfXcd = xcd * (K >> 3) + (xcd < (K & 7) ? xcd : (K & 7));
	const int countOfXcd = (K >> 3) + (xcd < (K & 7) ? 1 : 0);
	const bool nearAllowed = S2_WIDE_XCD_AFFINE && pv.nearHandoff != 0;
	const bool hopeLeft = nearAllowed && strip > firstOfXcd, hopeRight = nearAllowed && strip + 1 < firstOfXcd + countOfXcd;
	unsigned myXcc;
	asm volatile("s_getreg_b32 %0, hwreg(HW_REG_XCC_ID, 0, 4)" : "=s"(myXcc));
	constexpr unsigned epoch0 = 0u;
	if constexpr (SELF)
	{
		if (__builtin_amdgcn_readfirstlane(__hip_atomic_load(pv.deviceError, __ATOMIC_RELAXED, __HIP_MEMORY_SCOPE_AGENT)) != 0u)
		{
			return;
		}
	}
	gu64* census = (gu64*)pv.granules + pv.censusBase;
	if (S2_WIDE_XCD_AFFINE && tid == 0)
	{
		putGranule(census + strip, epoch0 + 1u, __uint_as_float(myXcc + 1u));
	}
	const StripDesc* da = ta.descs + strip;
	const PersistDesc* pd = pv.descs + strip;
	const int bodyBase = da->bodyBase, nb = da->bodyCount, roundsA = da->batchCount;
	constexpr int ROUNDS = 2 * RPH;
	constexpr int RA = ROUNDS + IL;
	static_assert(RA <= S2_STRIP_ROUNDS_MAX, "StripDesc::batch");
	int2 batchA[RA + 1];
	batchA[RA] = make_int2(0, 0);
#pragma unroll
	for (int i = 0; i < RA; ++i)
	{
		batchA[i] = make_int2(da->batch[i].x, da->batch[i].y);
	}
	const int nImp0 = pd->importCount[0], nImp1 = pd->importCount[1];
	const int roundsB0 = pd->seamBatchCount[0], roundsB1 = pd->seamBatchCount[1];
	constexpr int ST = SR + SL;
	static_assert(ST <= S2_PERSIST_B_ROUNDS, "PersistDesc::seamBatch");
	int2 batchB0[ST], batchB1[ST];
#pragma unroll
	for (int i = 0; i < ST; ++i)
	{
		batchB0[i] = pd->seamBatch[0][i];
		batchB1[i] = pd->seamBatch[1][i];
	}
	const int roundsB = roundsB0 > roundsB1 ? roundsB0 : roundsB1;
	const int nt = nb + nImp0 + nImp1;
	gu64* gran = (gu64*)pv.granules;
// ... 183 lines not shown
		seamMask |= mine ? 1u << i : 0u;
	}
#pragma unroll
	for (int i = SR; i < ST; ++i)
	{
		int seam, k;
		if (i < roundsB && seamItem(i, seam, k))
		{
			const int2 lb = c.localBodies[k];
			parkWide(lparked + (i - SR) * S2_WIDE_PARKED_RECORDS * sw, sw,
					 loadWide<RKP>(c, k, pv.remap[pd->remapBase[seam] + lb.x], pv.remap[pd->remapBase[seam] + lb.y]));
			seamMask |= 1u << i;
		}
	}
#pragma unroll
	for (int j = 0; j < IL; ++j)
	{
		const int k = kOfParked(j);
		if (k >= 0)
		{
			const int2 lb = c.localBodies[k];
			parkWide(lparkedI + j * S2_WIDE_PARKED_RECORDS * iw, iw, loadWide<RKP>(c, k, lb.x, lb.y));
		}
	}
	uint32_t flags[S2_WIDE_BODY_CHUNKS + 1];
	int ldsIdx[S2_WIDE_BODY_CHUNKS + 1];
#pragma unroll
	for (int ch = 0; ch < S2_WIDE_BODY_CHUNKS + 1; ++ch)
	{
		int gi = -1;
		if (ch < S2_WIDE_BODY_CHUNKS)
		{
			const int i = tid + ch * S2_WIDE_THREADS;
			ldsIdx[ch] = i;
			gi = i < nb ? (int)(id[ch] & ~S2G_OWNED) : -1;
		}
		else
		{
			ldsIdx[ch] = impSlotH;
			gi = impId;
		}
		flags[ch] = 0u;
		if (gi >= 0)
		{
			if constexpr (SELF)
			{
				const s2amdBody* w = self.wireBodies + gi;
				const int type = w->type;
				uint32_t f = 0x80000000u;
				if (type != S2AMD_BODY_FREE)
				{
					f |= S2F_LIVE | (type == S2AMD_BODY_DYNAMIC ? S2F_DYNAMIC : 0u) | (type != S2AMD_BODY_STATIC ? S2F_MOVES : 0u);
				}
				flags[ch] = f;
				const int i = ldsIdx[ch];
				lvel[i] = make_float4(w->linearVelocity[0], w->linearVelocity[1], w->angularVelocity, 0.0f);
				ldq[i] = make_float4(w->deltaPosition[0], w->deltaPosition[1], w->rot[0], w->rot[1]);
				if (ch < S2_WIDE_BODY_CHUNKS)
				{
					lpos[i] = make_float2(w->position[0], w->position[1]);
				}
				lmass[i] = make_float2(w->invMass, w->invI);
				const V2 gravity = v2(self.gravityX, self.gravityY);
				const V2 force = v2(w->force[0], w->force[1]);
				const V2 inner = mulAdd(force, w->mass * w->gravityScale, gravity);
				const V2 a = mulSV(self.unpackH * w->invMass, inner);
				const float aw = self.unpackH * w->invI * w->torque;
				const float ld = 1.0f / (1.0f + self.unpackH * w->linearDamping);
				const float ad = 1.0f / (1.0f + self.unpackH * w->angularDamping);
				linteg[i] = make_float4(a.x, a.y, aw, ld);
				langDamp[i] = ad;
			}
			else
			{
				lvel[ldsIdx[ch]] = g.vel[gi];
				ldq[ldsIdx[ch]] = g.dq[gi];
				flags[ch] = g.flags[gi] | 0x80000000u;
				linteg[ldsIdx[ch]] = g.integ[gi];
				langDamp[ldsIdx[ch]] = g.angDamp[gi];
				lmass[ldsIdx[ch]] = g.massInv[gi];
			}
		}
	}
	if constexpr (BODYWARM)
	{
		for (int i = tid; i < tw; i += S2_WIDE_THREADS)
		{
			lmask[i] = 0u;
		}
	}
	__shared__ int lovf[S2_OVERFLOW_BODIES];
	const int ovCount = OVERFLOW ? pv.overflowBodyCount : 0;
	if constexpr (OVERFLOW)
	{
		if (tid < S2_OVERFLOW_BODIES)
		{
			lovf[tid] = 0;
		}
		__syncthreads();
#pragma unroll
		for (int ch = 0; ch < S2_WIDE_BODY_CHUNKS + 1; ++ch)
		{
			if (flags[ch] != 0u)
			{
				const int gi = ch < S2_WIDE_BODY_CHUNKS ? (int)(id[ch] & ~S2G_OWNED) : impId;
				const int prio = ch < S2_WIDE_BODY_CHUNKS ? ((id[ch] & S2G_OWNED) != 0 ? 3 : 1) : 2;
				for (int m = 0; m < ovCount; ++m)
				{
					if (pv.overflowBodies[m] == gi)
					{
						atomicMax(&lovf[m], (prio << 24) | ldsIdx[ch]);
					}
				}
			}
		}
	}
	unsigned ovSweep = 0u;
	int* lnear = (int*)(lcoef + 2);
	if (ht == 0)
	{
		int near = 0;
		if (hopeH)
		{
			gu64* g = census + (half ? strip + 1 : strip - 1);
			for (int spins = 0; spins < 4096 && !near; ++spins)
			{
				const u64 x = __hip_atomic_load(g, __ATOMIC_RELAXED, __HIP_MEMORY_SCOPE_AGENT);
				if ((unsigned)(x >> 32) == epoch0 + 1u)
				{
					near = (unsigned)x == myXcc + 1u ? 1 : -1;
				}
			}
		}
		lnear[half] = near > 0 ? 1 : 0;
	}
	__syncthreads();
	const bool nearH = lnear[half] != 0;
	auto markStatic = [&](WideRegs& p) {
		const bool st = lmass[p.idx & 0x1fffu].x == 0.0f || lmass[(p.idx >> 13) & 0x1fffu].x == 0.0f;
		p.idx |= st ? 1u << 30 : 0u;
	};
#pragma unroll
	for (int s = 0; s < RPH; ++s)
	{
		if (kOfSlot(s) >= 0)
		{
			markStatic(rA[s]);
		}
	}
#pragma unroll
	for (int i = 0; i < SR; ++i)
	{
		if ((seamMask >> i) & 1u)
		{
			markStatic(rB[i]);
		}
	}
#pragma unroll
	for (int i = SR; i < ST; ++i)
	{
		if ((seamMask >> i) & 1u)
		{
			float4* slot = lparked + (i - SR) * S2_WIDE_PARKED_RECORDS * sw;
			WideRegs p = unparkWide(slot, sw);
			markStatic(p);
			slot[0].x = fromBits(p.idx);
		}
	}
#pragma unroll
	for (int j = 0; j < IL; ++j)
	{
		if (kOfParked(j) >= 0)
		{
			float4* slot = lparkedI + j * S2_WIDE_PARKED_RECORDS * iw;
			WideRegs p = unparkWide(slot, iw);
			markStatic(p);
			slot[0].x = fromBits(p.idx);
		}
	}
	if constexpr (BODYWARM)
	{
		auto note = [&](const WideRegs& p, int round) {
			const int ia = (int)(p.idx & 0x1fffu), ib = (int)((p.idx >> 13) & 0x1fffu);
			const uint32_t bit = (1u << round) | (((p.idx >> 26) & 3u) == 2u ? 1u << (16 + round) : 0u);
			if ((p.idx & (1u << 28)) != 0 && ia < nb)
			{
				atomicOr(&lmask[ia], bit);
			}
			if ((p.idx & (1u << 29)) != 0 && ib < nb)
			{
				atomicOr(&lmask[ib], bit);
			}
		};
#pragma unroll
		for (int s = 0; s < RPH; ++s)
		{
			if (kOfSlot(s) >= 0)
			{
				note(rA[s], 2 * s + half);
			}
		}
#pragma unroll
		for (int i = 0; i < SR; ++i)
		{
			if ((seamMask >> i) & 1u)
			{
				note(rB[i], ROUNDS + i);
			}
		}
		__syncthreads();
	}
	stampAt(1);

	unsigned epoch = epoch0;
	int bad = 0;
	for (int oi = 0; oi < opCount && !bad; ++oi)
	{
		const Op op = lops[oi];
		uint32_t salt;
		asm volatile("s_mov_b32 %0, 0" : "=s"(salt));
		if (op.code == OP_INTEGRATE_VEL)
		{
			if (BODYWARM && oi + 1 < opCount && lops[oi + 1].code == OP_WARM)
			{
				continue;
			}
#pragma unroll
			for (int ch = 0; ch < S2_WIDE_BODY_CHUNKS + 1; ++ch)
			{
				if ((flags[ch] & S2F_DYNAMIC) != 0)
				{
					const int i = ldsIdx[ch];
					float4 v = lvel[i], k = linteg[i];
					V2 lv = add(v2(v.x, v.y), v2(k.x, k.y));
					float w = v.z + k.z;
					lv = mulSV(k.w, lv);
					w *= langDamp[i];
					lvel[i] = make_float4(lv.x, lv.y, w, 0.0f);
				}
			}
			__syncthreads();
			stampAt(2);
		}
		else if (op.code == OP_INTEGRATE_POS)
		{
#pragma unroll
			for (int ch = 0; ch < S2_WIDE_BODY_CHUNKS + 1; ++ch)
			{
				if ((flags[ch] & S2F_MOVES) != 0)
				{
					const int i = ldsIdx[ch];
					float4 v = lvel[i], d = ldq[i];
					V2 dpos = mulAdd(v2(d.x, d.y), op.h, v2(v.x, v.y));
					Rot q;
					q.s = d.z, q.c = d.w;
					q = integrateRot(q, op.h * v.z);
					ldq[i] = make_float4(dpos.x, dpos.y, q.s, q.c);
				}
			}
			__syncthreads();
			stampAt(2);
		}
		else if (op.code == OP_FINALIZE)
		{
			const uint32_t need = op.flag ? S2F_DYNAMIC : S2F_MOVES;
#pragma unroll
			for (int ch = 0; ch < S2_WIDE_BODY_CHUNKS + 1; ++ch)
			{
				if ((flags[ch] & need) != 0)
				{
					const int i = ldsIdx[ch];
					const float4 d = ldq[i];
					if (ch < S2_WIDE_BODY_CHUNKS && (id[ch] & S2G_OWNED) != 0)
					{
						if constexpr (SELF)
						{
							const float2 pos = lpos[i];
							const V2 np = add(v2(pos.x, pos.y), v2(d.x, d.y));
							lpos[i] = make_float2(np.x, np.y);
						}
						else
						{
							const int gi = (int)(id[ch] & ~S2G_OWNED);
							const float2 pos = g.pos[gi];
							const V2 np = add(v2(pos.x, pos.y), v2(d.x, d.y));
							g.pos[gi] = make_float2(np.x, np.y);
						}
					}
					ldq[i] = make_float4(0.0f, 0.0f, d.z, d.w);
				}
			}
			__syncthreads();
			stampAt(2);
		}
		else if (BODYWARM && op.code == OP_WARM)
		{
#pragma unroll
			for (int s = 0; s < RPH; ++s)
			{
				if (kOfSlot(s) >= 0)
				{
					if (s >= LL0)
					{
						warmTermsWide<POINTS, true>(rA[s], ldq, lmass, lt, tw, TR, 2 * s + half, nb, salt, localsOf(s));
					}
					else
					{
						warmTermsWide<POINTS>(rA[s], ldq, lmass, lt, tw, TR, 2 * s + half, nb, salt);
					}
				}
			}
#pragma unroll
			for (int i = 0; i < SR; ++i)
			{
				if ((seamMask >> i) & 1u)
				{
					if (RPH + i >= LL0)
					{
						warmTermsWide<POINTS, true>(rB[i], ldq, lmass, lt, tw, TR, ROUNDS + i, nb, salt, localsOf(RPH + i));
					}
					else
					{
						warmTermsWide<POINTS>(rB[i], ldq, lmass, lt, tw, TR, ROUNDS + i, nb, salt);
					}
				}
			}
			__syncthreads();
			stampAt(15);
			const bool integrate = oi > 0 && lops[oi - 1].code == OP_INTEGRATE_VEL;
#pragma unroll
			for (int ch = 0; ch < S2_WIDE_BODY_CHUNKS; ++ch)
			{
				const int i = ldsIdx[ch];
				if (flags[ch] != 0u && i < nb)
				{
					const uint32_t m = lmask[i];
					const bool dynamic = integrate && (flags[ch] & S2F_DYNAMIC) != 0;
					if (m != 0u || dynamic)
					{
						const float4 v = lvel[i];
						V2 lv = v2(v.x, v.y);
						float w = v.z;
						if (dynamic)
						{
							const float4 k = linteg[i];
							lv = add(lv, v2(k.x, k.y));
							w = w + k.z;
							lv = mulSV(k.w, lv);
							w *= langDamp[i];
						}
						const int plane = TR * tw;
#pragma unroll
						for (int r = 0; r < TR; ++r)
						{
							if ((m >> r) & 1u)
							{
								const float2 t0 = lt[r * tw + i], t1 = lt[plane + r * tw + i], t2 = lt[2 * plane + r * tw + i];
								lv.x = lv.x + t0.x, lv.y = lv.y + t0.y, w = w + t1.x;
								if (POINTS == 2 || ((m >> (16 + r)) & 1u))
								{
									lv.x = lv.x + t1.y, lv.y = lv.y + t2.x, w = w + t2.y;
								}
							}
						}
						lvel[i] = make_float4(lv.x, lv.y, w, 0.0f);
					}
				}
			}
			__syncthreads();
			stampAt(3);
		}
		else if (op.code == OP_WARM)
		{
#pragma unroll
			for (int i = 0; i < ROUNDS; ++i)
			{
				if (i < roundsA)
				{
					if ((i & 1) == half && kOfSlot(i >> 1) >= 0)
					{
						if ((i >> 1) >= LL0)
						{
							warmWide<RK, POINTS, true>(rA[i >> 1], lvel, ldq, lmass, salt, nullptr, localsOf(i >> 1));
						}
						else
						{
							warmWide<RK, POINTS>(rA[i >> 1], lvel, ldq, lmass, salt, larms + 2 * (i >> 1) * S2_WIDE_THREADS);
						}
					}
					__syncthreads();
				}
			}
#pragma unroll
			for (int j = 0; j < IL; ++j)
			{
				if (ROUNDS + j < roundsA)
				{
					if (kOfParked(j) >= 0)
					{
						warmWide<RKP, POINTS>(unparkWide(lparkedI + j * S2_WIDE_PARKED_RECORDS * iw, iw), lvel, ldq, lmass, salt);
					}
					__syncthreads();
				}
			}
#pragma unroll
			for (int i = 0; i < SR; ++i)
			{
				if (i < roundsB)
				{
					if ((seamMask >> i) & 1u)
					{
						if (RPH + i >= LL0)
						{
							warmWide<RK, POINTS, true>(rB[i], lvel, ldq, lmass, salt, nullptr, localsOf(RPH + i));
						}
						else
						{
							warmWide<RK, POINTS>(rB[i], lvel, ldq, lmass, salt, larms + 2 * (RPH + i) * S2_WIDE_THREADS);
						}
					}
					__syncthreads();
				}
			}
#pragma unroll
			for (int i = SR; i < ST; ++i)
			{
				if (i < roundsB)
				{
					if ((seamMask >> i) & 1u)
					{
						warmWide<RKP, POINTS>(unparkWide(lparked + (i - SR) * S2_WIDE_PARKED_RECORDS * sw, sw), lvel, ldq, lmass, salt);
					}
					__syncthreads();
				}
			}
			if constexpr (OVERFLOW)
			{
				bad = wideOverflowExchange(pv, lovf, lvel, ovCount, ++ovSweep);
			}
			stampAt(3);
		}
		else if (op.code == OP_SOLVE_SOFT)
		{
			WidePrep pre;
			if (half == 0 && kOfSlot(0) >= 0)
			{
				if (0 >= LL0)
				{
					pre = prepWide<RK, POINTS, true>(rA[0], ldq, lcoef, op.inv_h, op.useBias, salt, nullptr, localsOf(0));
				}
				else
				{
					pre = prepWide<RK, POINTS>(rA[0], ldq, lcoef, op.inv_h, op.useBias, salt, larms);
				}
			}
#pragma unroll
			for (int i = 0; i < RA; ++i)
			{
				if (i < roundsA)
				{
					if ((i & 1) == half)
					{
						if (i < ROUNDS)
						{
							if (kOfSlot(i >> 1) >= 0)
							{
								chainWide<POINTS>(rA[i >> 1 < RPH ? i >> 1 : 0], pre, lvel, lmass, lcoef, salt);
							}
						}
						else if (kOfParked(i - ROUNDS < IL ? i - ROUNDS : 0) >= 0)
						{
							float4* slot = lparkedI + (i - ROUNDS) * S2_WIDE_PARKED_RECORDS * iw;
							WideRegs p = unparkWide(slot, iw);
							chainWide<POINTS>(p, pre, lvel, lmass, lcoef, salt);
							slot[5 * iw] = make_float4(p.imp[0].x, p.imp[0].y, p.imp[1].x, p.imp[1].y);
						}
					}
					else if (i + 1 < RA)
					{
						if (i + 1 < ROUNDS)
						{
							if (kOfSlot((i + 1) >> 1) >= 0)
							{
								if (((i + 1) >> 1) >= LL0)
								{
									pre = prepWide<RK, POINTS, true>(rA[(i + 1) >> 1 < RPH ? (i + 1) >> 1 : 0], ldq, lcoef, op.inv_h, op.useBias, salt, nullptr, localsOf((i + 1) >> 1));
								}
								else
								{
									pre = prepWide<RK, POINTS>(rA[(i + 1) >> 1 < RPH ? (i + 1) >> 1 : 0], ldq, lcoef, op.inv_h, op.useBias, salt, larms + 2 * ((i + 1) >> 1) * S2_WIDE_THREADS);
								}
							}
						}
						else if (kOfParked(i + 1 - ROUNDS < IL ? i + 1 - ROUNDS : 0) >= 0)
						{
							pre = prepWide<RKP, POINTS>(unparkWide(lparkedI + (i + 1 - ROUNDS) * S2_WIDE_PARKED_RECORDS * iw, iw), ldq, lcoef, op.inv_h, op.useBias, salt);
						}
					}
					__syncthreads();
					if (S2_PERSIST_INSTRUMENTED && i + 1 < roundsA && i < 6)
					{
						stampAt(8 + i);
					}
				}
			}
			stampAt(4);
			epoch += 1;
			const int par = (int)(epoch & 1u) * pv.parityStride;
			const bool mute = (pv.debugSkip & 8) != 0 && strip == 1;
			if (ht < nExpH && !mute)
			{
				const float4 v = lvel[expIdx];
				gu64* p = gran + par + outH + 4 * ht;
				if (nearH)
				{
					putGranuleNear(p + 0, epoch, v.x), putGranuleNear(p + 1, epoch, v.y), putGranuleNear(p + 2, epoch, v.z);
				}
				else
				{
					putGranule(p + 0, epoch, v.x), putGranule(p + 1, epoch, v.y), putGranule(p + 2, epoch, v.z);
				}
			}
			constexpr int SRP = SR < 2 ? SR : 2;
			WidePrep preB[SRP];
#pragma unroll
			for (int i = 0; i < SRP; ++i)
			{
				if ((seamMask >> i) & 1u)
				{
					if (RPH + i >= LL0)
					{
						preB[i] = prepWide<RK, POINTS, true>(rB[i], ldq, lcoef, op.inv_h, op.useBias, salt, nullptr, localsOf(RPH + i));
					}
					else
					{
						preB[i] = prepWide<RK, POINTS>(rB[i], ldq, lcoef, op.inv_h, op.useBias, salt, larms + 2 * (RPH + i) * S2_WIDE_THREADS);
					}
				}
			}
			WidePrep preP[SL > 0 ? SL : 1];
#pragma unroll
			for (int i = SR; i < ST; ++i)
			{
				if (S2_WIDE_PARKED_PREP_EARLY && ((seamMask >> i) & 1u))
				{
					preP[i - SR] = prepWide<RKP, POINTS>(unparkWide(lparked + (i - SR) * S2_WIDE_PARKED_RECORDS * sw, sw), ldq, lcoef, op.inv_h, op.useBias, salt);
				}
			}
			int fail = 0;
			if (ht < nImpH)
			{
				float v[3];
				if (getGranules<3>(gran + par + inH + 4 * ht, epoch, v, pv.error, pv.deviceError, pv.spinLimit))
				{
					lvel[impSlotH] = make_float4(v[0], v[1], v[2], 0.0f);
				}
				else
				{
					fail = 1;
				}
			}
			bad = __syncthreads_or(fail);
			if (bad)
			{
				break;
			}
			stampAt(5);
#pragma unroll
			for (int i = 0; i < SR; ++i)
			{
				if (i < roundsB)
				{
					if ((seamMask >> i) & 1u)
					{
						if constexpr (SR > 2)
						{
							if (i >= 2)
							{
								const WidePrep late = (RPH + i >= LL0) ? prepWide<RK, POINTS, true>(rB[i], ldq, lcoef, op.inv_h, op.useBias, salt, nullptr, localsOf(RPH + i))
																	   : prepWide<RK, POINTS>(rB[i], ldq, lcoef, op.inv_h, op.useBias, salt, larms + 2 * (RPH + i) * S2_WIDE_THREADS);
								chainWide<POINTS>(rB[i], late, lvel, lmass, lcoef, salt);
							}
							else
							{
								chainWide<POINTS>(rB[i], preB[i < 2 ? i : 0], lvel, lmass, lcoef, salt);
							}
						}
						else
						{
							chainWide<POINTS>(rB[i], preB[i], lvel, lmass, lcoef, salt);
						}
					}
					__syncthreads();
					if (S2_PERSIST_INSTRUMENTED && i + 1 < roundsB)
					{
						stampAt(14 + i);
					}
				}
			}
#pragma unroll
			for (int i = SR; i < ST; ++i)
			{
				if (i < roundsB)
// ... 144 lines not shown
			}
		}
	}
	else
	{
#pragma unroll
		for (int ch = 0; ch < S2_WIDE_BODY_CHUNKS; ++ch)
		{
			const int i = tid + ch * S2_WIDE_THREADS;
			if (i < nb && (id[ch] & S2G_OWNED) != 0)
			{
				const int gi = (int)(id[ch] & ~S2G_OWNED);
				g.vel[gi] = lvel[i];
				g.dq[gi] = ldq[i];
			}
		}
#pragma unroll
		for (int s = 0; s < RPH; ++s)
		{
			if (kOfSlot(s) >= 0)
			{
				storeWide(c, rA[s], kOfSlot(s));
			}
		}
#pragma unroll
		for (int j = 0; j < IL; ++j)
		{
			if (kOfParked(j) >= 0)
			{
				storeWide(c, unparkWide(lparkedI + j * S2_WIDE_PARKED_RECORDS * iw, iw), kOfParked(j));
			}
		}
#pragma unroll
		for (int i = 0; i < SR; ++i)
		{
			int seam, k;
			if (i < roundsB && seamItem(i, seam, k) && seam == 1)
			{
				storeWide(c, rB[i], k);
			}
		}
#pragma unroll
		for (int i = SR; i < ST; ++i)
		{
			int seam, k;
			if (i < roundsB && seamItem(i, seam, k) && seam == 1)
			{
				storeWide(c, unparkWide(lparked + (i - SR) * S2_WIDE_PARKED_RECORDS * sw, sw), k);
			}
		}
	}
	if constexpr (SLICED)
	{
		if (!bad)
		{
			if (ht < nImpH)
			{
#pragma unroll
				for (int par = 0; par < 2; ++par)
				{
					gu64* p = gran + par * pv.parityStride + inH + 4 * ht;
					p[0] = 0ull, p[1] = 0ull, p[2] = 0ull, p[3] = 0ull;
				}
			}
		}
	}
	stampAt(7);
	if (stamp)
	{
		pv.debugTimes[254] = 1ull;
		pv.debugTimes[255] = (unsigned long long)stamps;
	}
}

#ifndef S2_WIDE_ONLY_MAIN
#define S2_WIDE_ONLY_MAIN 0
#endif
#if S2_WIDE_ONLY_MAIN
template __global__ void wideStepKernel<2, 3, 2, 0, 0, 0>(ContactView, BodyView, StripTableView, PersistView, const Op*, int, WideSelf);
template __global__ void wideStepKernel<2, 3, 2, 0, 0, 1>(ContactView, BodyView, StripTableView, PersistView, const Op*, int, WideSelf);
template __global__ void wideStepKernel<2, 3, 2, 0, 0, 2>(ContactView, BodyView, StripTableView, PersistView, const Op*, int, WideSelf);
template __global__ void wideStepKernel<2, 3, 2, 0, 0, 3>(ContactView, BodyView, StripTableView, PersistView, const Op*, int, WideSelf);
template __global__ void wideStepKernel<2, 3, 2, 0, 0, 8>(ContactView, BodyView, StripTableView, PersistView, const Op*, int, WideSelf);
#else
template <int RPH, int SR, int SL, int IL, int MODE, int KIND = SOFT_TGS>
static void launchWideMode(hipStream_t s, dim3 grid, size_t lds, const ContactView& c, const BodyView& g, const StripTableView& a, const PersistView& pv, const Op* ops, int opCount,
						   const WideSelf& self)
{
	const dim3 block(S2_WIDE_THREADS);
	if (pv.allTwoPoints)
	{
		wideStepKernel<2, RPH, SR, SL, IL, MODE, KIND><<<grid, block, lds, s>>>(c, g, a, pv, ops, opCount, self);
	}
	else
	{
		wideStepKernel<0, RPH, SR, SL, IL, MODE, KIND><<<grid, block, lds, s>>>(c, g, a, pv, ops, opCount, self);
	}
}

static size_t wideExtraLds(const PersistView& pv, int RPH, int SR, int SL, int IL, bool selfContained, bool bodyWarm, bool fixedArms = false, bool tgsLocals = false)
{
	size_t records = (size_t)S2_WIDE_PARKED_RECORDS * ((size_t)SL * pv.parkSeamWidth + (size_t)IL * pv.parkInteriorWidth);
	records += fixedArms ? (size_t)2 * (RPH + SR) * S2_WIDE_THREADS : 0;
	records += tgsLocals ? (size_t)2 * wideLocalsInLds(RPH, SR, SL, IL, true) * S2_WIDE_THREADS : 0;
	records += selfContained ? (size_t)(pv.maxStaged + 1) / 2 : 0;
	if (bodyWarm)
	{
		const size_t tw = (size_t)pv.maxStripBodies, rounds = (size_t)(2 * RPH + SR);
		records += (tw + 3) / 4 + (3 * rounds * tw + 1) / 2;
	}
	return records * sizeof(float4);
}

template <int RPH, int SR, int SL = 0, int IL = 0>
static void launchWide(hipStream_t s, dim3 grid, size_t lds, const ContactView& c, const BodyView& g, const StripTableView& a, const PersistView& pv, const Op* ops, int opCount,
					   const WideSelf* self, int kind)
{
	if (kind == SOFT_FIXED)
	{
		if constexpr (RPH == 3 && SR == 2 && SL == 0 && IL == 0)
		{
			const WideSelf none{};
			lds += wideExtraLds(pv, RPH, SR, SL, IL, false, false, true);
			if (pv.overflowKernel != 0)
			{
				launchWideMode<RPH, SR, SL, IL, S2_WIDE_OVERFLOW, SOFT_FIXED>(s, grid, lds, c, g, a, pv, ops, opCount, none);
			}
			else if (pv.clearOwn != 0)
			{
				launchWideMode<RPH, SR, SL, IL, S2_WIDE_SLICED, SOFT_FIXED>(s, grid, lds, c, g, a, pv, ops, opCount, none);
			}
			else
			{
				launchWideMode<RPH, SR, SL, IL, 0, SOFT_FIXED>(s, grid, lds, c, g, a, pv, ops, opCount, none);
			}
		}
		return;
	}
	if (kind == SOFT_PGS)
	{
		const WideSelf none{};
		lds += wideExtraLds(pv, RPH, SR, SL, IL, false, false, true);
		if (pv.overflowKernel != 0)
		{
			launchWideMode<RPH, SR, SL, IL, S2_WIDE_OVERFLOW, SOFT_PGS>(s, grid, lds, c, g, a, pv, ops, opCount, none);
		}
		else if (pv.clearOwn != 0)
		{
			launchWideMode<RPH, SR, SL, IL, S2_WIDE_SLICED, SOFT_PGS>(s, grid, lds, c, g, a, pv, ops, opCount, none);
		}
		else
		{
			launchWideMode<RPH, SR, SL, IL, 0, SOFT_PGS>(s, grid, lds, c, g, a, pv, ops, opCount, none);
		}
		return;
	}
	constexpr bool OPTIONAL_MODES = RPH == 3 && SR == 2 && SL == 0 && IL == 0;
	const bool selfContained = OPTIONAL_MODES && self != nullptr;
	const bool bodyWarm = OPTIONAL_MODES && pv.bodyWarm != 0;
	lds += wideExtraLds(pv, RPH, SR, SL, IL, selfContained, bodyWarm, false, true);
	const WideSelf none{};
	if constexpr (OPTIONAL_MODES)
	{
		if (selfContained && bodyWarm && pv.allTwoPoints)
		{
			wideStepKernel<2, RPH, SR, SL, IL, S2_WIDE_SELF | S2_WIDE_BODYWARM><<<grid, dim3(S2_WIDE_THREADS), lds, s>>>(c, g, a, pv, ops, opCount, *self);
			return;
		}
		if (bodyWarm && !selfContained)
		{
			launchWideMode<RPH, SR, SL, IL, S2_WIDE_BODYWARM>(s, grid, lds, c, g, a, pv, ops, opCount, none);
			return;
		}
	}
	if constexpr (OPTIONAL_MODES)
	{
		if (selfContained)
		{
			launchWideMode<RPH, SR, SL, IL, S2_WIDE_SELF>(s, grid, lds, c, g, a, pv, ops, opCount, *self);
			return;
		}
	}
	{
		if (pv.overflowKernel != 0)
		{
			launchWideMode<RPH, SR, SL, IL, S2_WIDE_OVERFLOW>(s, grid, lds, c, g, a, pv, ops, opCount, none);
		}
		else if (pv.clearOwn != 0)
		{
			launchWideMode<RPH, SR, SL, IL, S2_WIDE_SLICED>(s, grid, lds, c, g, a, pv, ops, opCount, none);
		}
		else
		{
			launchWideMode<RPH, SR, SL, IL, 0>(s, grid, lds, c, g, a, pv, ops, opCount, none);
		}
	}
}

static int wideVariant(const PersistView& pv)
{
	if (pv.maxRoundsA > 8 || pv.maxSeamRounds > 4)
	{
		return -1;
	}
	const bool park = (pv.debugSkip & 16) != 0;
	if (park)
	{
		return pv.maxRoundsA <= 6 ? 3 : 4;
	}
	if (pv.maxRoundsA <= 6 && pv.maxSeamRounds <= 2)
	{
		return 0;
	}
	if (pv.maxRoundsA <= 6 && pv.maxSeamRounds <= 3)
	{
		return 1;
	}
	if (pv.maxSeamRounds <= 2)
	{
		return 2;
	}
	return pv.maxRoundsA <= 6 ? 3 : 4;
}

int wideExtraRecords(const PersistView& pv, int selfContained, int bodyWarm, int kind)
{
	static const int shape[5][4] = {{3, 2, 0, 0}, {3, 3, 0, 0}, {4, 2, 0, 0}, {3, 2, 2, 0}, {3, 2, 2, 2}};
	const int v = wideVariant(pv);
	if (v < 0 || (kind == SOFT_FIXED && v > 0) || ((selfContained != 0 || bodyWarm != 0) && v > 0))
	{
		return -1;
	}
	if (kind == SOFT_FIXED)
	{
		return (int)(wideExtraLds(pv, shape[v][0], shape[v][1], 0, 0, false, false, true) / sizeof(float4));
	}
	if (kind == SOFT_PGS)
	{
		return (int)(wideExtraLds(pv, shape[v][0], shape[v][1], shape[v][2], shape[v][3], false, false, true) / sizeof(float4));
	}
	const bool warm = bodyWarm != 0 && shape[v][2] == 0 && shape[v][3] == 0;
	return (int)(wideExtraLds(pv, shape[v][0], shape[v][1], shape[v][2], shape[v][3], selfContained != 0, warm, false, true) / sizeof(float4));
}

int wideBodyWarmVariant(const PersistView& pv)
{
	const int v = wideVariant(pv);
	return v == 0 ? 1 : 0;
}

void launchWideStep(hipStream_t s, int kind, const ContactView& c, const BodyView& g, const StripTableView& a, const PersistView& pv, const Op* ops, int opCount, const WideSelf* self)
{
	const dim3 grid((unsigned)a.groupCount + (pv.overflowKernel != 0 ? 1u : 0u));
	const size_t lds = (size_t)(pv.bodyRecords + 3) * sizeof(float4) + (size_t)opCount * sizeof(Op);
	switch (wideVariant(pv))
	{
		case 0:
			launchWide<3, 2>(s, grid, lds, c, g, a, pv, ops, opCount, self, kind);
			break;
		case 1:
			launchWide<3, 3>(s, grid, lds, c, g, a, pv, ops, opCount, self, kind);
			break;
		case 2:
			launchWide<4, 2>(s, grid, lds, c, g, a, pv, ops, opCount, self, kind);
			break;
		case 3:
			launchWide<3, 2, 2>(s, grid, lds, c, g, a, pv, ops, opCount, self, kind);
			break;
		case 4:
			launchWide<3, 2, 2, 2>(s, grid, lds, c, g, a, pv, ops, opCount, self, kind);
			break;
		default:
			break;
	}
}

constexpr int wideIslandLocalsInLds(int ROUNDS) { return ROUNDS > S2_STRIP_ROUNDS ? 6 : 0; }
int wideIslandLocalRecords(int maxRounds) { return 2 * wideIslandLocalsInLds(maxRounds > S2_STRIP_ROUNDS ? S2_STRIP_ROUNDS_MAX : S2_STRIP_ROUNDS) * S2_WIDE_THREADS; }

template <int ROUNDS, bool SELF, int POINTS>
__global__ __launch_bounds__(S2_WIDE_THREADS) void wideIslandKernel(ContactView c, BodyView g, StripTableView ta, float4 softCoef0, float4 softCoef1, const Op* ops,
																	 int opCount, s2amdContact* wire, s2amdBody* wireBodies, const uint32_t* hostFlags, int warmStart,
																	 StepConsts sc, float unpackH, const unsigned int* stepFailed)
{
	extern __shared__ __attribute__((aligned(16))) float4 lds[];
	if (stepFailed != nullptr && *stepFailed != 0u)
	{
		return;
	}
	const int tid = (int)threadIdx.x;
	const StripDesc* da = ta.descs + blockIdx.x;
	const int bodyBase = da->bodyBase, nb = da->bodyCount, roundsA = da->batchCount;
	int2 batchA[ROUNDS];
#pragma unroll
	for (int i = 0; i < ROUNDS; ++i)
	{
		batchA[i] = make_int2(da->batch[i].x, da->batch[i].y);
	}
	float4* lvel = lds;
	float4* ldq = lds + nb;
	float4* linteg = lds + 2 * nb;
	float* langDamp = (float*)(lds + 3 * nb);
	float2* lmass = (float2*)(lds + 3 * nb + (nb + 3) / 4);
	float2* llc = (float2*)(lds + 3 * nb + (nb + 3) / 4 + (nb + 1) / 2);
	const int bodyRecords = 3 * nb + (nb + 3) / 4 + 2 * ((nb + 1) / 2);
	Op* lops = (Op*)(lds + bodyRecords);
	float4* lcoef = lds + bodyRecords + 2 * opCount;
	constexpr int LA = wideIslandLocalsInLds(ROUNDS), LL0 = ROUNDS - LA;
	float4* llocals = lcoef + 2 + tid;
	auto localsOf = [&](int r) { return llocals + 2 * (r - LL0 > 0 ? r - LL0 : 0) * S2_WIDE_THREADS; };

	uint32_t id[S2_STRIP_BODY_CHUNKS];
#pragma unroll
	for (int ch = 0; ch < S2_STRIP_BODY_CHUNKS; ++ch)
	{
		const int i = tid + ch * S2_WIDE_THREADS;
		id[ch] = i < nb ? (uint32_t)ta.bodyIds[bodyBase + i] : 0u;
	}
	for (int i = tid; i < opCount * 8; i += S2_WIDE_THREADS)
	{
		((int*)lops)[i] = ((const int*)ops)[i];
	}
	if (tid < 2)
	{
		lcoef[tid] = tid ? softCoef1 : softCoef0;
	}
	auto kOfRound = [&](int i) {
		const int k = batchA[i].x + tid;
		return (i < roundsA && k < batchA[i].y) ? k : -1;
	};
	int slotOf[ROUNDS];
	int2 localOf[ROUNDS];
#pragma unroll
	for (int i = 0; i < ROUNDS; ++i)
	{
		slotOf[i] = -1;
		localOf[i] = make_int2(0, 0);
		if (kOfRound(i) >= 0)
		{
			slotOf[i] = c.contactIndex[kOfRound(i)];
			localOf[i] = c.localBodies[kOfRound(i)];
		}
	}
	uint32_t flags[S2_STRIP_BODY_CHUNKS];
	float2 pos[S2_STRIP_BODY_CHUNKS];
#pragma unroll
	for (int ch = 0; ch < S2_STRIP_BODY_CHUNKS; ++ch)
	{
		const int i = tid + ch * S2_WIDE_THREADS;
		flags[ch] = 0u;
		pos[ch] = make_float2(0.0f, 0.0f);
		if (i < nb)
		{
			const int gi = (int)(id[ch] & ~S2G_OWNED);
			if constexpr (SELF)
			{
// ... 326 lines not shown
```

solver2d_amd/hip.py:

```python
import ctypes
import os

import numpy as np

from . import wire

_HERE = os.path.dirname(os.path.abspath(__file__))
LIB_PATH = os.environ.get("S2AMD_LIB") or os.path.join(_HERE, "libs2amd.so")
FAST_LIB_PATH = os.environ.get("S2AMD_FAST_LIB") or os.path.join(_HERE, "libs2amd_fast.so")

EXPORTS = [
    "s2amd_api_version", "s2amd_build_flags", "s2amd_device_count", "s2amd_device_bus_id", "s2amd_last_error", "s2amd_create", "s2amd_destroy",
    "s2amd_solve", "s2amd_upload", "s2amd_step_resident", "s2amd_download", "s2amd_save_bodies",
    "s2amd_restore_bodies", "s2amd_get_contact_order", "s2amd_get_joint_order", "s2amd_get_writable_bodies", "s2amd_get_stats",
    "s2amd_set_option", "s2amd_export_poses", "s2amd_export_poses_async", "s2amd_export_bodies_async", "s2amd_export_wait", "s2amd_measure_dominant", "s2amd_refit_shapes", "s2amd_find_pairs", "s2amd_synchronize", "s2amd_update_contacts", "s2amd_find_islands", "s2amd_color_constraints",
    "s2amd_world_upload", "s2amd_world_step", "s2amd_world_download", "s2amd_world_find_pairs", "s2amd_world_set_contacts",
    "s2amd_device_alloc", "s2amd_device_free", "s2amd_device_read", "s2amd_world_separated", "s2amd_world_download_boxes", "s2amd_world_set_refit_order", "s2amd_world_download_step", "s2amd_world_set_tree", "s2amd_world_get_tree",
    "s2amd_get_strip_owners",
    "s2amd_sharded_create", "s2amd_sharded_destroy", "s2amd_sharded_shard_count", "s2amd_sharded_solver", "s2amd_sharded_upload", "s2amd_sharded_step",
    "s2amd_sharded_download", "s2amd_sharded_read_bodies", "s2amd_sharded_reshard", "s2amd_sharded_get_partition",
    "s2amd_sharded_step_async", "s2amd_sharded_wait", "s2amd_sharded_get_step_ops", "s2amd_sharded_count_ops",
]

_libs = {}


class S2AmdError(RuntimeError):
    pass


def load(fast=False):
    path = FAST_LIB_PATH if fast else LIB_PATH
    if path in _libs:
        return _libs[path]
    if not os.path.exists(path):
        raise S2AmdError("HIP extension %s is missing: build it with `make -C solver2d_amd/csrc` "
                         "(there is no CPU fallback)" % path)
    L = ctypes.CDLL(path)
    vp, i32 = ctypes.c_void_p, ctypes.c_int32
    L.s2amd_api_version.restype = ctypes.c_int
    L.s2amd_device_count.restype = ctypes.c_int
    L.s2amd_last_error.restype = ctypes.c_char_p
    L.s2amd_build_flags.restype = ctypes.c_char_p
    L.s2amd_create.argtypes = [ctypes.c_int, ctypes.POINTER(vp)]
    L.s2amd_destroy.argtypes = [vp]
    L.s2amd_destroy.restype = None
    L.s2amd_solve.argtypes = [vp, ctypes.POINTER(wire.StepParams), vp, i32, vp, i32, vp, i32]
    L.s2amd_upload.argtypes = [vp, vp, i32, vp, i32, vp, i32]
    L.s2amd_step_resident.argtypes = [vp, ctypes.POINTER(wire.StepParams)]
    L.s2amd_download.argtypes = [vp, vp, i32, vp, i32, vp, i32]
    L.s2amd_save_bodies.argtypes = [vp]
    L.s2amd_restore_bodies.argtypes = [vp]
    L.s2amd_synchronize.argtypes = [vp]
    L.s2amd_get_contact_order.argtypes = [vp, vp, i32, vp, i32, ctypes.POINTER(i32), ctypes.POINTER(i32)]
    L.s2amd_get_joint_order.argtypes = [vp, vp, i32, vp, i32, ctypes.POINTER(i32), ctypes.POINTER(i32)]
    L.s2amd_get_writable_bodies.argtypes = [vp, vp, i32, ctypes.POINTER(i32)]
    L.s2amd_get_strip_owners.argtypes = [vp, vp, vp, i32, ctypes.POINTER(i32)]
    L.s2amd_get_stats.argtypes = [vp, ctypes.POINTER(wire.StepStats)]
    L.s2amd_set_option.argtypes = [vp, ctypes.c_char_p, i32]
    L.s2amd_export_poses.argtypes = [vp, vp, i32]
    L.s2amd_export_poses_async.argtypes = [vp, vp, i32, i32]
    L.s2amd_export_bodies_async.argtypes = [vp, vp, i32, i32]
    L.s2amd_export_wait.argtypes = [vp, i32]
    L.s2amd_measure_dominant.argtypes = [vp, ctypes.POINTER(wire.StepParams), i32, ctypes.POINTER(ctypes.c_float),
                                         ctypes.POINTER(i32), ctypes.POINTER(i32)]
    L.s2amd_refit_shapes.argtypes = [vp, vp, i32, vp, i32, vp]
    L.s2amd_find_pairs.argtypes = [vp, vp, i32, vp, i32, vp, vp, i32, vp, i32, vp, i32, ctypes.POINTER(i32)]
    L.s2amd_update_contacts.argtypes = [vp, vp, i32, vp, vp, i32, vp, vp, i32, vp]
    L.s2amd_world_upload.argtypes = [vp, vp, i32, vp, i32, vp, i32, vp, i32, vp, vp]
    L.s2amd_world_step.argtypes = [vp, ctypes.POINTER(wire.StepParams), ctypes.POINTER(wire.WorldStepInfo)]
    L.s2amd_world_find_pairs.argtypes = [vp, vp, i32, ctypes.POINTER(i32)]
    L.s2amd_world_set_contacts.argtypes = [vp, vp, i32, vp, vp]
    L.s2amd_world_separated.argtypes = [vp, vp, i32, ctypes.POINTER(i32)]
    L.s2amd_world_download_boxes.argtypes = [vp, vp, i32]
    L.s2amd_world_set_refit_order.argtypes = [vp, vp, i32]
    L.s2amd_world_set_tree.argtypes = [vp, i32, vp, i32, i32]
    L.s2amd_world_get_tree.argtypes = [vp, i32, vp, i32, ctypes.POINTER(i32)]
    L.s2amd_world_download.argtypes = [vp, vp, i32, vp, i32, vp, i32, vp, i32, vp, vp, vp]
    L.s2amd_device_alloc.argtypes = [vp, ctypes.c_uint64, ctypes.POINTER(vp)]
    L.s2amd_device_free.argtypes = [vp, vp]
    L.s2amd_device_read.argtypes = [vp, vp, vp, ctypes.c_uint64]
    L.s2amd_find_islands.argtypes = [vp, vp, i32, vp, i32, vp, i32, vp, ctypes.POINTER(i32)]
    L.s2amd_color_constraints.argtypes = [vp, vp, i32, vp, i32, vp, ctypes.POINTER(i32), ctypes.POINTER(i32)]
    L.s2amd_sharded_create.argtypes = [vp, i32, ctypes.POINTER(vp)]
    L.s2amd_sharded_destroy.argtypes = [vp]
    L.s2amd_sharded_destroy.restype = None
    L.s2amd_sharded_shard_count.argtypes = [vp]
    L.s2amd_sharded_solver.argtypes = [vp, i32]
    L.s2amd_sharded_solver.restype = vp
    L.s2amd_sharded_upload.argtypes = [vp, vp, i32, vp, i32, vp, i32]
    L.s2amd_sharded_step.argtypes = [vp, ctypes.POINTER(wire.StepParams)]
    L.s2amd_sharded_step_async.argtypes = [vp, ctypes.POINTER(wire.StepParams)]
    L.s2amd_sharded_wait.argtypes = [vp]
    L.s2amd_sharded_get_step_ops.argtypes = [vp, ctypes.POINTER(i32), ctypes.POINTER(i32), ctypes.POINTER(i32)]
    L.s2amd_sharded_count_ops.argtypes = [i32, i32, ctypes.POINTER(i32)]
    L.s2amd_sharded_download.argtypes = [vp, vp, i32, vp, i32, vp, i32]
    L.s2amd_sharded_read_bodies.argtypes = [vp, i32, vp, i32]
    L.s2amd_sharded_reshard.argtypes = [vp, vp, i32, vp, i32]
    L.s2amd_sharded_get_partition.argtypes = [vp, vp, i32, ctypes.POINTER(i32), ctypes.POINTER(i32)]
    if L.s2amd_api_version() != wire.API_VERSION:
        raise S2AmdError("libs2amd.so API version %d != %d" % (L.s2amd_api_version(), wire.API_VERSION))
    if fast and not L.s2amd_build_flags().decode().count("contract=fast"):
        raise S2AmdError("%s is not a tolerance-mode build (%s)" % (path, L.s2amd_build_flags().decode()))
    _libs[path] = L
    return L


def device_count():
    return load().s2amd_device_count()


def device_bus_id(device):
    buf = ctypes.create_string_buffer(64)
    _check(load().s2amd_device_bus_id(int(device), buf, 64))
    return buf.value.decode()


def _check(rc, L=None):
    if rc != 0:
        raise S2AmdError("s2amd error %d: %s" % (rc, (L or load()).s2amd_last_error().decode(errors="replace")))


_env_options_logged = False


def env_options():
    global _env_options_logged
    text = os.environ.get("S2AMD_OPTIONS", "")
    out = []
    for kv in filter(None, (e.strip() for e in text.split(","))):
        k, eq, v = kv.partition("=")
        try:
            if not eq or not k.strip():
                raise ValueError
            out.append((k.strip(), int(v)))
        except ValueError:
            raise S2AmdError("S2AMD_OPTIONS: entry %r is not key=integer" % kv) from None
    if out and not _env_options_logged:
        import sys
        print("[s2amd] S2AMD_OPTIONS applied to every solver: %s" % ", ".join("%s=%d" % e for e in out), file=sys.stderr)
        _env_options_logged = True
# ... 166 lines not shown
    def world_separated(self, expected=64):
        out = np.zeros(max(int(expected), 1), dtype=np.int32)
        n = ctypes.c_int32()
        rc = self._L.s2amd_world_separated(self._h, wire.as_ptr(out), len(out), ctypes.byref(n))
        if rc == -5:
            out = np.zeros(n.value, dtype=np.int32)
            rc = self._L.s2amd_world_separated(self._h, wire.as_ptr(out), len(out), ctypes.byref(n))
        self._ck(rc)
        return out[: n.value].copy()

    def world_set_contacts(self, slots, contacts, pairs):
        slots = np.ascontiguousarray(slots, dtype=np.int32)
        contacts = np.ascontiguousarray(contacts)
        pairs = np.ascontiguousarray(pairs)
        assert contacts.dtype == wire.contact_dtype and pairs.dtype == wire.pair_state_dtype and len(slots) == len(contacts) == len(pairs)
        self._ck(self._L.s2amd_world_set_contacts(self._h, wire.as_ptr(slots), len(slots), wire.as_ptr(contacts), wire.as_ptr(pairs)))

    def world_download(self, bodies, contacts, joints, shapes, pairs, origins):
        origins = np.ascontiguousarray(origins, dtype=np.float32)
        status = np.zeros(len(contacts), dtype=np.int32)
        self._ck(self._L.s2amd_world_download(self._h, *self._args(bodies, contacts, joints), wire.as_ptr(shapes), len(shapes), wire.as_ptr(pairs),
                                           wire.as_ptr(origins), wire.as_ptr(status)))
        return bodies, contacts, joints, shapes, pairs, origins, status

    def find_islands(self, bodies, contacts, joints):
        island = np.full(len(bodies), -2, dtype=np.int32)
        n = ctypes.c_int32()
        self._ck(self._L.s2amd_find_islands(self._h, wire.as_ptr(bodies), len(bodies), wire.as_ptr(contacts), len(contacts), wire.as_ptr(joints),
                                         len(joints), wire.as_ptr(island), ctypes.byref(n)))
        return island, n.value

    def color_constraints(self, bodies, contacts):
        colour = np.full(len(contacts), -2, dtype=np.int32)
        n, r = ctypes.c_int32(), ctypes.c_int32()
        self._ck(self._L.s2amd_color_constraints(self._h, wire.as_ptr(bodies), len(bodies), wire.as_ptr(contacts), len(contacts), wire.as_ptr(colour),
                                              ctypes.byref(n), ctypes.byref(r)))
        return colour, n.value, r.value

    def find_pairs(self, bodies, shapes, moved, existing, joints):
        existing = np.ascontiguousarray(existing, dtype=np.int32).reshape(-1, 2)
        moved = np.ascontiguousarray(moved, dtype=np.uint8)
        cap = 4096
        while True:
            out = np.zeros((cap, 2), dtype=np.int32)
            n = ctypes.c_int32()
            rc = self._L.s2amd_find_pairs(self._h, wire.as_ptr(bodies), len(bodies), wire.as_ptr(shapes), len(shapes), wire.as_ptr(moved),
                                         wire.as_ptr(existing), len(existing), wire.as_ptr(joints), len(joints), wire.as_ptr(out), cap,
                                         ctypes.byref(n))
            if rc == -5 and n.value > cap:
                cap = n.value
                continue
            self._ck(rc)
            return out[: n.value].copy()

    def _order(self, fn):
        n, nc = ctypes.c_int32(), ctypes.c_int32()
        self._ck(fn(self._h, None, 0, None, 0, ctypes.byref(n), ctypes.byref(nc)))
        order = np.zeros(max(n.value, 1), dtype=np.int32)
        offsets = np.zeros(nc.value + 1, dtype=np.int32)
        self._ck(fn(self._h, order.ctypes.data, len(order), offsets.ctypes.data, len(offsets), ctypes.byref(n), ctypes.byref(nc)))
        return order[: n.value].copy(), offsets

    def contact_order(self):
        return self._order(self._L.s2amd_get_contact_order)

    def strip_owners(self, body_capacity):
        owner = np.full(max(body_capacity, 1), -1, dtype=np.int32)
        seam = np.full(max(body_capacity, 1), -1, dtype=np.int32)
        n = ctypes.c_int32()
        self._ck(self._L.s2amd_get_strip_owners(self._h, owner.ctypes.data, seam.ctypes.data, len(owner), ctypes.byref(n)))
        return owner[:body_capacity], seam[:body_capacity], n.value

    def joint_order(self):
        return self._order(self._L.s2amd_get_joint_order)

    def synchronize(self):
        self._ck(self._L.s2amd_synchronize(self._h))

    def stats(self):
        st = wire.StepStats()
        self._ck(self._L.s2amd_get_stats(self._h, ctypes.byref(st)))
        return {k: getattr(st, k) for k, _ in wire.StepStats._fields_}


class _BorrowedSolver(Solver):

    def __init__(self, L, handle):
        self._L, self._h, self.fast = L, ctypes.c_void_p(handle), False

    def close(self):
        self._h = None


class ShardedSolver:

    def __init__(self, devices, fast=False):
        L = load(fast=fast)
        devs = (ctypes.c_int32 * len(devices))(*[int(d) for d in devices])
        h = ctypes.c_void_p()
        _check(L.s2amd_sharded_create(devs, len(devices), ctypes.byref(h)), L)
        self._L, self._h = L, h
        self.shards = len(devices)
        self.body_capacity = 0

    def close(self):
        if getattr(self, "_h", None):
            self._L.s2amd_sharded_destroy(self._h)
            self._h = None

    def __del__(self):
        try:
            self.close()
        except Exception:
            pass

    def __enter__(self):
        return self

    def __exit__(self, *a):
        self.close()

    def _ck(self, rc):
        _check(rc, self._L)

    def shard(self, i):
        h = self._L.s2amd_sharded_solver(self._h, int(i))
        if not h:
            raise S2AmdError("no shard %d" % i)
        return _BorrowedSolver(self._L, h)

    def upload(self, bodies, contacts, joints):
        self._ck(self._L.s2amd_sharded_upload(self._h, *Solver._args(bodies, contacts, joints)))
        self.body_capacity = len(bodies)

    def step(self, params):
        self._ck(self._L.s2amd_sharded_step(self._h, ctypes.byref(params)))

    def step_async(self, params):
        self._ck(self._L.s2amd_sharded_step_async(self._h, ctypes.byref(params)))

    def wait(self):
        self._ck(self._L.s2amd_sharded_wait(self._h))

    def step_ops(self):
        ops, waits, ex = ctypes.c_int32(), ctypes.c_int32(), ctypes.c_int32()
        self._ck(self._L.s2amd_sharded_get_step_ops(self._h, ctypes.byref(ops), ctypes.byref(waits), ctypes.byref(ex)))
        return ops.value, waits.value, ex.value

    def download(self, bodies, contacts, joints):
        self._ck(self._L.s2amd_sharded_download(self._h, *Solver._args(bodies, contacts, joints)))
        return bodies, contacts, joints

    def read_bodies(self, shard=0):
        out = np.zeros((self.body_capacity, 8), dtype=np.float32)
        self._ck(self._L.s2amd_sharded_read_bodies(self._h, int(shard), wire.as_ptr(out.reshape(-1)), self.body_capacity))
        return out

    def reshard(self, contacts=None, joints=None):
        for arr, dt in ((contacts, wire.contact_dtype), (joints, wire.joint_dtype)):
            if arr is not None and (arr.dtype != dt or not arr.flags["C_CONTIGUOUS"]):
                raise ValueError("array must be a contiguous %s array" % (dt.names,))
        self._ck(self._L.s2amd_sharded_reshard(self._h, wire.as_ptr(contacts) if contacts is not None else None, len(contacts) if contacts is not None else 0,
                                               wire.as_ptr(joints) if joints is not None else None, len(joints) if joints is not None else 0))

    def partition(self):
        out = np.full(max(self.body_capacity, 1), -1, dtype=np.int32)
# ... 4 lines not shown
```

Before: 6.248 billion.

## Fold warm-start terms into the final relax round in wide TGS_Soft kernel

Adds a relax-fed warm-start mode to the wide persistent kernel. When a non-biased soft solve is followed by velocity integration and a warm op, the relax sweep now writes per-body warm-start impulse terms to LDS while it still holds the prepared constraint data. The separate integrate pass is skipped and the warm op applies the terms together with integration. This is meant to save a full pass over the constraints and a barrier per substep, at the cost of extra LDS and a new kernel variant. The mode is on by default and a getter reports which wide mode ran.

After: 6.341 billion (median of 6 runs). 1.01x the previous value.

```diff
diff --git a/include/solver2d_amd.h b/include/solver2d_amd.h
--- a/include/solver2d_amd.h
+++ b/include/solver2d_amd.h
@@ -284,6 +284,7 @@
 						  int32_t colorCapacity, int32_t* jointCount, int32_t* colorCount);
 int s2amd_get_writable_bodies(s2amdSolver* solver, uint8_t* writable, int32_t bodyCapacity, int32_t* solverClass);
 int s2amd_get_stats(s2amdSolver* solver, s2amdStepStats* stats);
+int s2amd_get_wide_mode(s2amdSolver* solver, int32_t* mode);
 int s2amd_get_strip_owners(s2amdSolver* solver, int32_t* ownerStrip, int32_t* onSeam, int32_t capacity, int32_t* stripCount);
 int s2amd_measure_dominant(s2amdSolver* solver, const s2amdStepParams* params, int32_t repeats, float* usPerLaunch,
 						   int32_t* launchesPerSweep, int32_t* constraintsPerLaunch);
diff --git a/solver2d_amd/csrc/launch.h b/solver2d_amd/csrc/launch.h
--- a/solver2d_amd/csrc/launch.h
+++ b/solver2d_amd/csrc/launch.h
@@ -162,7 +162,7 @@
 void launchWideIsland(hipStream_t s, const ContactView& c, const BodyView& g, const StripTableView& t, const float4* softCoef, const Op* ops, int opCount,
 					  int maxRounds, s2amdContact* wire, s2amdBody* wireBodies, const uint32_t* hostFlags, int warmStart, const StepConsts& sc, float unpackH,
 					  int selfContained, const unsigned int* stepFailed, int allTwoPoints);
-void launchWideStep(hipStream_t s, int kind, const ContactView& c, const BodyView& g, const StripTableView& a, const PersistView& pv, const Op* ops, int opCount,
+int launchWideStep(hipStream_t s, int kind, const ContactView& c, const BodyView& g, const StripTableView& a, const PersistView& pv, const Op* ops, int opCount,
 					const WideSelf* self);
 
 int jacobiKernelSetup();
diff --git a/solver2d_amd/csrc/s2_device.h b/solver2d_amd/csrc/s2_device.h
--- a/solver2d_amd/csrc/s2_device.h
+++ b/solver2d_amd/csrc/s2_device.h
@@ -497,6 +497,7 @@
 	int maxStaged;
 	int maxStripBodies;
 	int bodyWarm;
+	int relaxWarm;
 	int clearOwn;
 	const int* overflowBodies;
 	int overflowBodyCount;
diff --git a/solver2d_amd/csrc/solver.cpp b/solver2d_amd/csrc/solver.cpp
--- a/solver2d_amd/csrc/solver.cpp
+++ b/solver2d_amd/csrc/solver.cpp
@@ -659,6 +659,16 @@
 	return S2AMD_OK;
 }
 
+int s2amd_get_wide_mode(s2amdSolver* s, int32_t* mode)
+{
+	if (!s || !mode)
+	{
+		return fail(S2AMD_E_INVALID, "null argument");
+	}
+	*mode = s->stepWideMode;
+	return S2AMD_OK;
+}
+
 int s2amd_export_poses(s2amdSolver* s, void* devicePoses, int32_t capacity)
 {
 	if (!s || !s->resident)
@@ -1091,6 +1101,10 @@
 	{
 		s->optWideBodyWarm = value != 0;
 	}
+	else if (strcmp(key, "relax_warm_terms") == 0)
+	{
+		s->optWideRelaxWarm = value != 0;
+	}
 	else if (strcmp(key, "self_contained_strips") == 0)
 	{
 		if (s->optSelfContainedStrips != (value != 0 ? 1 : 0))
diff --git a/solver2d_amd/csrc/solver_executor.h b/solver2d_amd/csrc/solver_executor.h
--- a/solver2d_amd/csrc/solver_executor.h
+++ b/solver2d_amd/csrc/solver_executor.h
@@ -442,6 +442,11 @@
 		return s->optWideBodyWarm != 0 && wideBodyWarmVariant(s->persist) != 0 && wideFits(selfContained, true);
 	}
 
+	bool wideRelaxWarm() const
+	{
+		return s->optWideRelaxWarm != 0 && wideBodyWarmVariant(s->persist) != 0 && wideFits(false, true);
+	}
+
 	bool residentPlan(int& kind, int& warm) const
 	{
 		kind = -1, warm = -1;
@@ -629,7 +634,7 @@
 		{
 			pv.ldsRecords = s->persistRecordsWide;
 		}
-		pv.bodyWarm = 0;
+		pv.bodyWarm = 0, pv.relaxWarm = 0;
 		pv.clearOwn = 1;
 		const IncrementalStrips& m = s->stripInc;
 		int first = 0;
@@ -641,7 +646,7 @@
 			{
 				continue;
 			}
-			launchWideStep(st, kind, s->cv, s->bv, s->leanA, pv, (const Op*)s->dPersistOps.p + first, i + 1 - first, nullptr);
+			s->wideMode = launchWideStep(st, kind, s->cv, s->bv, s->leanA, pv, (const Op*)s->dPersistOps.p + first, i + 1 - first, nullptr);
 			count();
 			if (sweep)
 			{
@@ -692,15 +697,16 @@
 				self.warmStart = p.sc.warmStart, self.gravityX = p.sc.gravityX, self.gravityY = p.sc.gravityY, self.unpackH = p.unpackH;
 			}
 			pv.bodyWarm = (kind == SOFT_TGS && wideBodyWarm(selfContained)) ? 1 : 0;
+			pv.relaxWarm = (kind == SOFT_TGS && !pv.bodyWarm && !selfContained && wideRelaxWarm()) ? 1 : 0;
 			if (overflowKernel)
 			{
 				const IncrementalStrips& m = s->stripInc;
-				pv.bodyWarm = 0;
+				pv.bodyWarm = 0, pv.relaxWarm = 0;
 				pv.overflowKernel = 1;
 				pv.overflowBodyCount = (int)m.overflowBodyIds.size();
 				pv.overflowBegin = m.overflowBegin, pv.overflowEnd = m.overflowEnd;
 			}
-			launchWideStep(st, kind, s->cv, s->bv, s->leanA, pv, (const Op*)s->dPersistOps.p, s->persistOpCount, selfContained ? &self : nullptr);
+			s->wideMode = launchWideStep(st, kind, s->cv, s->bv, s->leanA, pv, (const Op*)s->dPersistOps.p, s->persistOpCount, selfContained ? &self : nullptr);
 		}
 		else if (pv.pairLanes && s->optPairLanes)
 		{
diff --git a/solver2d_amd/csrc/solver_internal.h b/solver2d_amd/csrc/solver_internal.h
--- a/solver2d_amd/csrc/solver_internal.h
+++ b/solver2d_amd/csrc/solver_internal.h
@@ -306,6 +306,8 @@
 	int persistRecordsWide = 0;
 	DevBuf dPersistOps;
 	int persistOpCount = 0;
+	int wideMode = -1;
+	int stepWideMode = -1;
 	DevBuf dJacobi, dJacobiGran;
 	JacobiView jacobi{};
 	int jacobiDeferred = 0;
@@ -422,6 +424,7 @@
 	int optSeamRegs = 1;
 	int optWide = 1;
 	int optWideBodyWarm = 0;
+	int optWideRelaxWarm = 1;
 	int optSelfContainedStrips = 0;
 	int optStripSlack = 1;
 	int optPairLanes = 0;
diff --git a/solver2d_amd/csrc/solver_step.cpp b/solver2d_amd/csrc/solver_step.cpp
--- a/solver2d_amd/csrc/solver_step.cpp
+++ b/solver2d_amd/csrc/solver_step.cpp
@@ -681,6 +681,7 @@
 		const bool persistent = s->stats.persistent && q.persistPlan(kind, warm);
 		const bool wide = persistent && q.widePlan(kind, warm);
 		s->stats.pairLanes = wide ? 2 : (persistent && s->persist.pairLanes && s->optPairLanes) ? 1 : (s->stats.persistent && !persistent) ? 3 : 0;
+		s->stepWideMode = wide ? s->wideMode : -1;
 	}
 	s->stats.potentialConstraints = (int32_t)(s->contacts.order.size() - (size_t)s->slackPositions);
 	if (!async && s->hostError && *s->hostError != 0u)
diff --git a/solver2d_amd/csrc/wide_kernel.hip b/solver2d_amd/csrc/wide_kernel.hip
--- a/solver2d_amd/csrc/wide_kernel.hip
+++ b/solver2d_amd/csrc/wide_kernel.hip
@@ -481,6 +481,7 @@
 
 #define S2_WIDE_SELF 1
 #define S2_WIDE_BODYWARM 2
+#define S2_WIDE_RELAXWARM 16
 #define S2_WIDE_SLICED 4
 
 template <int POINTS, bool LL = false>
@@ -536,6 +537,88 @@
 	}
 }
 
+template <int POINTS>
+S2_DEV void warmTermsRelax(const WideRegs& p, const WidePrep& pre, const float2* lmass, float2* lt, int tw, int R, int round, int nOwn, uint32_t salt)
+{
+	const uint32_t idx = p.idx ^ salt;
+	const int ia = (int)(idx & 0x1fffu), ib = (int)((idx >> 13) & 0x1fffu);
+	const int pointCount = (int)((idx >> 26) & 3u);
+	const bool wa = (idx & (1u << 28)) != 0 && ia < nOwn, wb = (idx & (1u << 29)) != 0 && ib < nOwn;
+	const float2 mA = lmass[ia], mB = lmass[ib];
+	const V2 normal = v2(fromBits(asBits(p.n.x) ^ salt), p.n.y);
+	const V2 tangent = rightPerp(normal);
+	float tA[6], tB[6];
+#pragma unroll
+	for (int j = 0; j < 2; ++j)
+	{
+		tA[3 * j] = tA[3 * j + 1] = tA[3 * j + 2] = 0.0f;
+		tB[3 * j] = tB[3 * j + 1] = tB[3 * j + 2] = 0.0f;
+		if (POINTS == 2 || j < pointCount)
+		{
+#if S2_WIDE_PACKED
+			const V2 rA = v2(pre.pA[j].y, -pre.pA[j].x), rB = v2(pre.pB[j].y, -pre.pB[j].x);
+#else
+			const V2 rA = pre.rA[j], rB = pre.rB[j];
+#endif
+			const V2 P = add(mulSV(p.imp[j].x, normal), mulSV(p.imp[j].y, tangent));
+			tA[3 * j] = -mA.x * P.x, tA[3 * j + 1] = -mA.x * P.y, tA[3 * j + 2] = -(mA.y * cross(rA, P));
+			tB[3 * j] = mB.x * P.x, tB[3 * j + 1] = mB.x * P.y, tB[3 * j + 2] = mB.y * cross(rB, P);
+		}
+	}
+	float2* row = lt + (size_t)round * tw;
+	const int plane = R * tw;
+	if (wa)
+	{
+		row[ia] = make_float2(tA[0], tA[1]);
+		row[plane + ia] = make_float2(tA[2], tA[3]);
+		row[2 * plane + ia] = make_float2(tA[4], tA[5]);
+	}
+	if (wb)
+	{
+		row[ib] = make_float2(tB[0], tB[1]);
+		row[plane + ib] = make_float2(tB[2], tB[3]);
+		row[2 * plane + ib] = make_float2(tB[4], tB[5]);
+	}
+}
+
+S2_DEV int relaxWarmFlag(const Op* ops, int opCount, int j, int flag)
+{
+	auto next = [&](int k) {
+		do
+		{
+			++k;
+		} while (k < opCount && ops[k].code == OP_JOINT_SWEEP);
+		return k;
+	};
+	auto prev = [&](int k) {
+		do
+		{
+			--k;
+		} while (k >= 0 && ops[k].code == OP_JOINT_SWEEP);
+		return k;
+	};
+	auto folds = [&](int r) {
+		if (r < 0 || ops[r].code != OP_SOLVE_SOFT || ops[r].useBias != 0)
+		{
+			return 0;
+		}
+		const int v = next(r);
+		const int w = v < opCount ? next(v) : opCount;
+		return (w < opCount && ops[v].code == OP_INTEGRATE_VEL && ops[w].code == OP_WARM) ? 1 : 0;
+	};
+	switch (ops[j].code)
+	{
+		case OP_SOLVE_SOFT:
+			return folds(j);
+		case OP_INTEGRATE_VEL:
+			return folds(prev(j));
+		case OP_WARM:
+			return prev(j) >= 0 ? folds(prev(prev(j))) : 0;
+		default:
+			return flag;
+	}
+}
+
 constexpr int wideLocalsInLds(int RPH, int SR, int SL, int IL, bool sliced)
 {
 	const int plain = (SL > 0 || IL > 0) ? (IL > 0 ? 4 : 3) : ((RPH + SR > 5) ? 3 : 0);
@@ -761,6 +844,9 @@
 	static_assert(KIND == SOFT_TGS || (MODE & ~(S2_WIDE_SLICED | S2_WIDE_OVERFLOW)) == 0, "the self-contained form and the body-centric warm start are s2Solve_TGS_Soft's");
 	static_assert(!SLICED || MODE == S2_WIDE_SLICED, "a sliced step's launches are the plain form");
 	static_assert(!OVERFLOW || MODE == S2_WIDE_OVERFLOW, "the overflow workgroup rides with the plain form");
+	constexpr bool RELAXWARM = (MODE & S2_WIDE_RELAXWARM) != 0;
+	static_assert(!RELAXWARM || (MODE == S2_WIDE_RELAXWARM && SL == 0 && IL == 0), "the relax-fed warm start: the plain form, no parked rounds");
+	constexpr bool TERMS = BODYWARM || RELAXWARM;
 	if constexpr (OVERFLOW)
 	{
 		if (blockIdx.x + 1u == gridDim.x)
@@ -1110,7 +1196,7 @@
 			}
 		}
 	}
-	if constexpr (BODYWARM)
+	if constexpr (TERMS)
 	{
 		for (int i = tid; i < tw; i += S2_WIDE_THREADS)
 		{
@@ -1164,6 +1250,10 @@
 	}
 	__syncthreads();
 	const bool nearH = lnear[half] != 0;
+	for (int j = tid; RELAXWARM && j < opCount; j += S2_WIDE_THREADS)
+	{
+		lops[j].flag = relaxWarmFlag(lops, opCount, j, lops[j].flag);
+	}
 	auto markStatic = [&](WideRegs& p) {
 		const bool st = lmass[p.idx & 0x1fffu].x == 0.0f || lmass[(p.idx >> 13) & 0x1fffu].x == 0.0f;
 		p.idx |= st ? 1u << 30 : 0u;
@@ -1206,7 +1296,7 @@
 			slot[0].x = fromBits(p.idx);
 		}
 	}
-	if constexpr (BODYWARM)
+	if constexpr (TERMS)
 	{
 		auto note = [&](const WideRegs& p, int round) {
 			const int ia = (int)(p.idx & 0x1fffu), ib = (int)((p.idx >> 13) & 0x1fffu);
@@ -1239,7 +1329,6 @@
 		__syncthreads();
 	}
 	stampAt(1);
-
 	unsigned epoch = epoch0;
 	int bad = 0;
 	for (int oi = 0; oi < opCount && !bad; ++oi)
@@ -1250,6 +1339,10 @@
 		if (op.code == OP_INTEGRATE_VEL)
 		{
 			if (BODYWARM && oi + 1 < opCount && lops[oi + 1].code == OP_WARM)
+			{
+				continue;
+			}
+			if (RELAXWARM && lops[oi].flag != 0)
 			{
 				continue;
 			}
@@ -1321,41 +1414,56 @@
 			__syncthreads();
 			stampAt(2);
 		}
-		else if (BODYWARM && op.code == OP_WARM)
-		{
-#pragma unroll
-			for (int s = 0; s < RPH; ++s)
-			{
-				if (kOfSlot(s) >= 0)
-				{
-					if (s >= LL0)
-					{
-						warmTermsWide<POINTS, true>(rA[s], ldq, lmass, lt, tw, TR, 2 * s + half, nb, salt, localsOf(s));
-					}
-					else
-					{
-						warmTermsWide<POINTS>(rA[s], ldq, lmass, lt, tw, TR, 2 * s + half, nb, salt);
-					}
-				}
-			}
-#pragma unroll
-			for (int i = 0; i < SR; ++i)
-			{
-				if ((seamMask >> i) & 1u)
-				{
-					if (RPH + i >= LL0)
-					{
-						warmTermsWide<POINTS, true>(rB[i], ldq, lmass, lt, tw, TR, ROUNDS + i, nb, salt, localsOf(RPH + i));
-					}
-					else
+		else if (op.code == OP_WARM && (BODYWARM || (RELAXWARM && lops[oi].flag != 0)))
+		{
+			if constexpr (BODYWARM)
+			{
+#pragma unroll
+				for (int s = 0; s < RPH; ++s)
+				{
+					if (kOfSlot(s) >= 0)
+					{
+						if (s >= LL0)
+						{
+							warmTermsWide<POINTS, true>(rA[s], ldq, lmass, lt, tw, TR, 2 * s + half, nb, salt, localsOf(s));
+						}
+						else
+						{
+							warmTermsWide<POINTS>(rA[s], ldq, lmass, lt, tw, TR, 2 * s + half, nb, salt);
+						}
+					}
+				}
+#pragma unroll
+				for (int i = 0; i < SR; ++i)
+				{
+					if ((seamMask >> i) & 1u)
+					{
+						if (RPH + i >= LL0)
+						{
+							warmTermsWide<POINTS, true>(rB[i], ldq, lmass, lt, tw, TR, ROUNDS + i, nb, salt, localsOf(RPH + i));
+						}
+						else
+						{
+							warmTermsWide<POINTS>(rB[i], ldq, lmass, lt, tw, TR, ROUNDS + i, nb, salt);
+						}
+					}
+				}
+				__syncthreads();
+				stampAt(15);
+			}
+			else
+			{
+#pragma unroll
+				for (int i = 0; i < SR; ++i)
+				{
+					if ((seamMask >> i) & 1u)
 					{
 						warmTermsWide<POINTS>(rB[i], ldq, lmass, lt, tw, TR, ROUNDS + i, nb, salt);
 					}
 				}
-			}
-			__syncthreads();
-			stampAt(15);
-			const bool integrate = oi > 0 && lops[oi - 1].code == OP_INTEGRATE_VEL;
+				__syncthreads();
+			}
+			const bool integrate = RELAXWARM || (oi > 0 && lops[oi - 1].code == OP_INTEGRATE_VEL);
 #pragma unroll
 			for (int ch = 0; ch < S2_WIDE_BODY_CHUNKS; ++ch)
 			{
@@ -1471,6 +1579,7 @@
 		else if (op.code == OP_SOLVE_SOFT)
 		{
 			WidePrep pre;
+			const bool emit = RELAXWARM && lops[oi].flag != 0;
 			if (half == 0 && kOfSlot(0) >= 0)
 			{
 				if (0 >= LL0)
@@ -1504,25 +1613,32 @@
 							slot[5 * iw] = make_float4(p.imp[0].x, p.imp[0].y, p.imp[1].x, p.imp[1].y);
 						}
 					}
-					else if (i + 1 < RA)
-					{
-						if (i + 1 < ROUNDS)
+					else
+					{
+						if (RELAXWARM && emit && i >= 1 && i - 1 < ROUNDS && kOfSlot((i - 1) >> 1) >= 0)
 						{
-							if (kOfSlot((i + 1) >> 1) >= 0)
+							warmTermsRelax<POINTS>(rA[(i - 1) >> 1 < RPH ? (i - 1) >> 1 : 0], pre, lmass, lt, tw, TR, i - 1, nb, salt);
+						}
+						if (i + 1 < RA)
+						{
+							if (i + 1 < ROUNDS)
 							{
-								if (((i + 1) >> 1) >= LL0)
+								if (kOfSlot((i + 1) >> 1) >= 0)
 								{
-									pre = prepWide<RK, POINTS, true>(rA[(i + 1) >> 1 < RPH ? (i + 1) >> 1 : 0], ldq, lcoef, op.inv_h, op.useBias, salt, nullptr, localsOf((i + 1) >> 1));
-								}
-								else
-								{
-									pre = prepWide<RK, POINTS>(rA[(i + 1) >> 1 < RPH ? (i + 1) >> 1 : 0], ldq, lcoef, op.inv_h, op.useBias, salt, larms + 2 * ((i + 1) >> 1) * S2_WIDE_THREADS);
+									if (((i + 1) >> 1) >= LL0)
+									{
+										pre = prepWide<RK, POINTS, true>(rA[(i + 1) >> 1 < RPH ? (i + 1) >> 1 : 0], ldq, lcoef, op.inv_h, op.useBias, salt, nullptr, localsOf((i + 1) >> 1));
+									}
+									else
+									{
+										pre = prepWide<RK, POINTS>(rA[(i + 1) >> 1 < RPH ? (i + 1) >> 1 : 0], ldq, lcoef, op.inv_h, op.useBias, salt, larms + 2 * ((i + 1) >> 1) * S2_WIDE_THREADS);
+									}
 								}
 							}
-						}
-						else if (kOfParked(i + 1 - ROUNDS < IL ? i + 1 - ROUNDS : 0) >= 0)
-						{
-							pre = prepWide<RKP, POINTS>(unparkWide(lparkedI + (i + 1 - ROUNDS) * S2_WIDE_PARKED_RECORDS * iw, iw), ldq, lcoef, op.inv_h, op.useBias, salt);
+							else if (kOfParked(i + 1 - ROUNDS < IL ? i + 1 - ROUNDS : 0) >= 0)
+							{
+								pre = prepWide<RKP, POINTS>(unparkWide(lparkedI + (i + 1 - ROUNDS) * S2_WIDE_PARKED_RECORDS * iw, iw), ldq, lcoef, op.inv_h, op.useBias, salt);
+							}
 						}
 					}
 					__syncthreads();
@@ -1547,6 +1663,17 @@
 				else
 				{
 					putGranule(p + 0, epoch, v.x), putGranule(p + 1, epoch, v.y), putGranule(p + 2, epoch, v.z);
+				}
+			}
+			if (RELAXWARM && emit)
+			{
+#pragma unroll
+				for (int s = 0; s < RPH; ++s)
+				{
+					if (2 * s + half == roundsA - 1 && kOfSlot(s) >= 0)
+					{
+						warmTermsRelax<POINTS>(rA[s], pre, lmass, lt, tw, TR, 2 * s + half, nb, salt);
+					}
 				}
 			}
 			constexpr int SRP = SR < 2 ? SR : 2;
@@ -1857,9 +1984,10 @@
 template __global__ void wideStepKernel<2, 3, 2, 0, 0, 2>(ContactView, BodyView, StripTableView, PersistView, const Op*, int, WideSelf);
 template __global__ void wideStepKernel<2, 3, 2, 0, 0, 3>(ContactView, BodyView, StripTableView, PersistView, const Op*, int, WideSelf);
 template __global__ void wideStepKernel<2, 3, 2, 0, 0, 8>(ContactView, BodyView, StripTableView, PersistView, const Op*, int, WideSelf);
+template __global__ void wideStepKernel<2, 3, 2, 0, 0, 16>(ContactView, BodyView, StripTableView, PersistView, const Op*, int, WideSelf);
 #else
 template <int RPH, int SR, int SL, int IL, int MODE, int KIND = SOFT_TGS>
-static void launchWideMode(hipStream_t s, dim3 grid, size_t lds, const ContactView& c, const BodyView& g, const StripTableView& a, const PersistView& pv, const Op* ops, int opCount,
+static int launchWideMode(hipStream_t s, dim3 grid, size_t lds, const ContactView& c, const BodyView& g, const StripTableView& a, const PersistView& pv, const Op* ops, int opCount,
 						   const WideSelf& self)
 {
 	const dim3 block(S2_WIDE_THREADS);
@@ -1871,6 +1999,7 @@
 	{
 		wideStepKernel<0, RPH, SR, SL, IL, MODE, KIND><<<grid, block, lds, s>>>(c, g, a, pv, ops, opCount, self);
 	}
+	return MODE;
 }
 
 static size_t wideExtraLds(const PersistView& pv, int RPH, int SR, int SL, int IL, bool selfContained, bool bodyWarm, bool fixedArms = false, bool tgsLocals = false)
@@ -1888,7 +2017,7 @@
 }
 
 template <int RPH, int SR, int SL = 0, int IL = 0>
-static void launchWide(hipStream_t s, dim3 grid, size_t lds, const ContactView& c, const BodyView& g, const StripTableView& a, const PersistView& pv, const Op* ops, int opCount,
+static int launchWide(hipStream_t s, dim3 grid, size_t lds, const ContactView& c, const BodyView& g, const StripTableView& a, const PersistView& pv, const Op* ops, int opCount,
 					   const WideSelf* self, int kind)
 {
 	if (kind == SOFT_FIXED)
@@ -1899,18 +2028,18 @@
 			lds += wideExtraLds(pv, RPH, SR, SL, IL, false, false, true);
 			if (pv.overflowKernel != 0)
 			{
-				launchWideMode<RPH, SR, SL, IL, S2_WIDE_OVERFLOW, SOFT_FIXED>(s, grid, lds, c, g, a, pv, ops, opCount, none);
+				return launchWideMode<RPH, SR, SL, IL, S2_WIDE_OVERFLOW, SOFT_FIXED>(s, grid, lds, c, g, a, pv, ops, opCount, none);
 			}
 			else if (pv.clearOwn != 0)
 			{
-				launchWideMode<RPH, SR, SL, IL, S2_WIDE_SLICED, SOFT_FIXED>(s, grid, lds, c, g, a, pv, ops, opCount, none);
+				return launchWideMode<RPH, SR, SL, IL, S2_WIDE_SLICED, SOFT_FIXED>(s, grid, lds, c, g, a, pv, ops, opCount, none);
 			}
 			else
 			{
-				launchWideMode<RPH, SR, SL, IL, 0, SOFT_FIXED>(s, grid, lds, c, g, a, pv, ops, opCount, none);
-			}
-		}
-		return;
+				return launchWideMode<RPH, SR, SL, IL, 0, SOFT_FIXED>(s, grid, lds, c, g, a, pv, ops, opCount, none);
+			}
+		}
+		return -1;
 	}
 	if (kind == SOFT_PGS)
 	{
@@ -1918,56 +2047,59 @@
 		lds += wideExtraLds(pv, RPH, SR, SL, IL, false, false, true);
 		if (pv.overflowKernel != 0)
 		{
-			launchWideMode<RPH, SR, SL, IL, S2_WIDE_OVERFLOW, SOFT_PGS>(s, grid, lds, c, g, a, pv, ops, opCount, none);
+			return launchWideMode<RPH, SR, SL, IL, S2_WIDE_OVERFLOW, SOFT_PGS>(s, grid, lds, c, g, a, pv, ops, opCount, none);
 		}
 		else if (pv.clearOwn != 0)
 		{
-			launchWideMode<RPH, SR, SL, IL, S2_WIDE_SLICED, SOFT_PGS>(s, grid, lds, c, g, a, pv, ops, opCount, none);
+			return launchWideMode<RPH, SR, SL, IL, S2_WIDE_SLICED, SOFT_PGS>(s, grid, lds, c, g, a, pv, ops, opCount, none);
 		}
 		else
 		{
-			launchWideMode<RPH, SR, SL, IL, 0, SOFT_PGS>(s, grid, lds, c, g, a, pv, ops, opCount, none);
-		}
-		return;
+			return launchWideMode<RPH, SR, SL, IL, 0, SOFT_PGS>(s, grid, lds, c, g, a, pv, ops, opCount, none);
+		}
 	}
 	constexpr bool OPTIONAL_MODES = RPH == 3 && SR == 2 && SL == 0 && IL == 0;
 	const bool selfContained = OPTIONAL_MODES && self != nullptr;
 	const bool bodyWarm = OPTIONAL_MODES && pv.bodyWarm != 0;
-	lds += wideExtraLds(pv, RPH, SR, SL, IL, selfContained, bodyWarm, false, true);
+	const bool relaxWarm = OPTIONAL_MODES && !bodyWarm && !selfContained && pv.relaxWarm != 0 && pv.allTwoPoints && pv.overflowKernel == 0 && pv.clearOwn == 0;
+	lds += wideExtraLds(pv, RPH, SR, SL, IL, selfContained, bodyWarm || relaxWarm, false, true);
 	const WideSelf none{};
 	if constexpr (OPTIONAL_MODES)
 	{
+		if (relaxWarm)
+		{
+			wideStepKernel<2, RPH, SR, SL, IL, S2_WIDE_RELAXWARM><<<grid, dim3(S2_WIDE_THREADS), lds, s>>>(c, g, a, pv, ops, opCount, none);
+			return S2_WIDE_RELAXWARM;
+		}
 		if (selfContained && bodyWarm && pv.allTwoPoints)
 		{
 			wideStepKernel<2, RPH, SR, SL, IL, S2_WIDE_SELF | S2_WIDE_BODYWARM><<<grid, dim3(S2_WIDE_THREADS), lds, s>>>(c, g, a, pv, ops, opCount, *self);
-			return;
+			return S2_WIDE_SELF | S2_WIDE_BODYWARM;
 		}
 		if (bodyWarm && !selfContained)
 		{
-			launchWideMode<RPH, SR, SL, IL, S2_WIDE_BODYWARM>(s, grid, lds, c, g, a, pv, ops, opCount, none);
-			return;
+			return launchWideMode<RPH, SR, SL, IL, S2_WIDE_BODYWARM>(s, grid, lds, c, g, a, pv, ops, opCount, none);
 		}
 	}
 	if constexpr (OPTIONAL_MODES)
 	{
 		if (selfContained)
 		{
-			launchWideMode<RPH, SR, SL, IL, S2_WIDE_SELF>(s, grid, lds, c, g, a, pv, ops, opCount, *self);
-			return;
+			return launchWideMode<RPH, SR, SL, IL, S2_WIDE_SELF>(s, grid, lds, c, g, a, pv, ops, opCount, *self);
 		}
 	}
 	{
 		if (pv.overflowKernel != 0)
 		{
-			launchWideMode<RPH, SR, SL, IL, S2_WIDE_OVERFLOW>(s, grid, lds, c, g, a, pv, ops, opCount, none);
+			return launchWideMode<RPH, SR, SL, IL, S2_WIDE_OVERFLOW>(s, grid, lds, c, g, a, pv, ops, opCount, none);
 		}
 		else if (pv.clearOwn != 0)
 		{
-			launchWideMode<RPH, SR, SL, IL, S2_WIDE_SLICED>(s, grid, lds, c, g, a, pv, ops, opCount, none);
+			return launchWideMode<RPH, SR, SL, IL, S2_WIDE_SLICED>(s, grid, lds, c, g, a, pv, ops, opCount, none);
 		}
 		else
 		{
-			launchWideMode<RPH, SR, SL, IL, 0>(s, grid, lds, c, g, a, pv, ops, opCount, none);
+			return launchWideMode<RPH, SR, SL, IL, 0>(s, grid, lds, c, g, a, pv, ops, opCount, none);
 		}
 	}
 }
@@ -2024,29 +2156,24 @@
 	return v == 0 ? 1 : 0;
 }
 
-void launchWideStep(hipStream_t s, int kind, const ContactView& c, const BodyView& g, const StripTableView& a, const PersistView& pv, const Op* ops, int opCount, const WideSelf* self)
+int launchWideStep(hipStream_t s, int kind, const ContactView& c, const BodyView& g, const StripTableView& a, const PersistView& pv, const Op* ops, int opCount, const WideSelf* self)
 {
 	const dim3 grid((unsigned)a.groupCount + (pv.overflowKernel != 0 ? 1u : 0u));
 	const size_t lds = (size_t)(pv.bodyRecords + 3) * sizeof(float4) + (size_t)opCount * sizeof(Op);
 	switch (wideVariant(pv))
 	{
 		case 0:
-			launchWide<3, 2>(s, grid, lds, c, g, a, pv, ops, opCount, self, kind);
-			break;
+			return launchWide<3, 2>(s, grid, lds, c, g, a, pv, ops, opCount, self, kind);
 		case 1:
-			launchWide<3, 3>(s, grid, lds, c, g, a, pv, ops, opCount, self, kind);
-			break;
+			return launchWide<3, 3>(s, grid, lds, c, g, a, pv, ops, opCount, self, kind);
 		case 2:
-			launchWide<4, 2>(s, grid, lds, c, g, a, pv, ops, opCount, self, kind);
-			break;
+			return launchWide<4, 2>(s, grid, lds, c, g, a, pv, ops, opCount, self, kind);
 		case 3:
-			launchWide<3, 2, 2>(s, grid, lds, c, g, a, pv, ops, opCount, self, kind);
-			break;
+			return launchWide<3, 2, 2>(s, grid, lds, c, g, a, pv, ops, opCount, self, kind);
 		case 4:
-			launchWide<3, 2, 2, 2>(s, grid, lds, c, g, a, pv, ops, opCount, self, kind);
-			break;
+			return launchWide<3, 2, 2, 2>(s, grid, lds, c, g, a, pv, ops, opCount, self, kind);
 		default:
-			break;
+			return -1;
 	}
 }
 
diff --git a/solver2d_amd/hip.py b/solver2d_amd/hip.py
--- a/solver2d_amd/hip.py
+++ b/solver2d_amd/hip.py
@@ -12,7 +12,7 @@
 EXPORTS = [
     "s2amd_api_version", "s2amd_build_flags", "s2amd_device_count", "s2amd_device_bus_id", "s2amd_last_error", "s2amd_create", "s2amd_destroy",
     "s2amd_solve", "s2amd_upload", "s2amd_step_resident", "s2amd_download", "s2amd_save_bodies",
-    "s2amd_restore_bodies", "s2amd_get_contact_order", "s2amd_get_joint_order", "s2amd_get_writable_bodies", "s2amd_get_stats",
+    "s2amd_restore_bodies", "s2amd_get_contact_order", "s2amd_get_joint_order", "s2amd_get_writable_bodies", "s2amd_get_stats", "s2amd_get_wide_mode",
     "s2amd_set_option", "s2amd_export_poses", "s2amd_export_poses_async", "s2amd_export_bodies_async", "s2amd_export_wait", "s2amd_measure_dominant", "s2amd_refit_shapes", "s2amd_find_pairs", "s2amd_synchronize", "s2amd_update_contacts", "s2amd_find_islands", "s2amd_color_constraints",
     "s2amd_world_upload", "s2amd_world_step", "s2amd_world_download", "s2amd_world_find_pairs", "s2amd_world_set_contacts",
     "s2amd_device_alloc", "s2amd_device_free", "s2amd_device_read", "s2amd_world_separated", "s2amd_world_download_boxes", "s2amd_world_set_refit_order", "s2amd_world_download_step", "s2amd_world_set_tree", "s2amd_world_get_tree",
@@ -57,6 +57,7 @@
     L.s2amd_get_writable_bodies.argtypes = [vp, vp, i32, ctypes.POINTER(i32)]
     L.s2amd_get_strip_owners.argtypes = [vp, vp, vp, i32, ctypes.POINTER(i32)]
     L.s2amd_get_stats.argtypes = [vp, ctypes.POINTER(wire.StepStats)]
+    L.s2amd_get_wide_mode.argtypes = [vp, ctypes.POINTER(ctypes.c_int32)]
     L.s2amd_set_option.argtypes = [vp, ctypes.c_char_p, i32]
     L.s2amd_export_poses.argtypes = [vp, vp, i32]
     L.s2amd_export_poses_async.argtypes = [vp, vp, i32, i32]
@@ -389,6 +390,11 @@
         self._ck(self._L.s2amd_get_stats(self._h, ctypes.byref(st)))
         return {k: getattr(st, k) for k, _ in wire.StepStats._fields_}
 
+    def wide_mode(self):
+        m = ctypes.c_int32(-1)
+        self._ck(self._L.s2amd_get_wide_mode(self._h, ctypes.byref(m)))
+        return m.value
+
 
 class _BorrowedSolver(Solver):
 
```
